# B-R-P/NMSLIB-ZIG

Measured on AMD Instinct MI355X. Metric: queries/sec @ recall@10, 1M x 128-D L2, batch=1024; HBM GB/s vs peak, higher is better.
Workload: dtype f16+f32

## Files before the change

include/nmslib_gpu.h:

```cpp
#ifndef NMSLIB_GPU_H
#define NMSLIB_GPU_H

#include "nmslib_c.h"

#ifdef __cplusplus
extern "C" {
#endif

int nmslib_gpu_device_count(void);

nmslib_error_t nmslib_gpu_finalize(nmslib_index_handle_t index);

nmslib_error_t nmslib_gpu_knn_query_batch_device(nmslib_index_handle_t index,
                                                 const void* d_queries, size_t query_count,
                                                 size_t elem_count, size_t k, int32_t* d_ids,
                                                 float* d_dists, int32_t* d_counts,
                                                 void* stream);

nmslib_error_t nmslib_gpu_last_batch_counters(nmslib_index_handle_t index,
                                              const int32_t** d_ndc, const int32_t** d_hops,
                                              const int32_t** d_hops_up);

nmslib_error_t nmslib_gpu_merge_topk(const float* d_dists_in, const int32_t* d_ids_in,
                                     size_t nshards, size_t query_count, size_t k,
                                     float* d_dists_out, int32_t* d_ids_out, void* stream);

nmslib_error_t nmslib_gpu_merge_topk_strided(const float* d_dists_in, const int32_t* d_ids_in,
                                             size_t shard_stride, size_t nshards, size_t query_count,
                                             size_t k, float* d_dists_out, int32_t* d_ids_out,
                                             void* stream);

nmslib_error_t nmslib_gpu_kernel_timing(nmslib_index_handle_t index, int enable, double* total_ms,
                                        uint64_t* launches);

typedef struct {
    double upload_seconds;
    double build_seconds;
    size_t hbm_bytes;
    size_t rows;
    size_t dim;
    size_t shards;
    size_t last_path;
    size_t fast_tiles;
    size_t fast_tiles_precise;
    size_t fast_tiles_fallback;
    size_t hnsw_redone;
} nmslib_gpu_stats_t;
nmslib_error_t nmslib_gpu_get_stats(nmslib_index_handle_t index, nmslib_gpu_stats_t* out);

nmslib_error_t nmslib_gpu_graph_builder(nmslib_index_handle_t index, int* builder);

nmslib_error_t nmslib_gpu_string_hnsw_links(nmslib_index_handle_t index, size_t node, int level, int32_t* out,
                                            size_t capacity, size_t* count, int* enterpoint, int* maxlevel);

#ifdef __cplusplus
}
#endif
#endif
```

nmslib_zig_amd/__init__.py:

```python
import ctypes as C
import os
import subprocess

import numpy as np

_HERE = os.path.dirname(os.path.abspath(__file__))
LIB_PATH = os.path.join(_HERE, "libnmslib_c.so")

ERRORS = {
    1: "NullPointer", 2: "InvalidArgument", 3: "OutOfMemory", 4: "BufferTooSmall",
    5: "SpaceIncompatible", 6: "QueryTooLarge", 7: "InvalidSparseElement", 8: "IndexBuildFailed",
    9: "QueryExecutionFailed", 10: "DataIOFailed", 11: "PluginRegistrationFailed", 12: "Internal",
    13: "Runtime", 14: "IndexNotBuilt",
}
DATATYPE = {"DenseVector": 0, "SparseVector": 1, "DenseUInt8Vector": 2, "ObjectAsString": 3}
DISTTYPE = {"Float": 0, "Int": 1}
SPARSE_ELEM = np.dtype([("id", "<u4"), ("value", "<f4")])


def sparse_rows(rows):
    if hasattr(rows, "indptr"):
        rows = (rows.indptr, rows.indices, rows.data)
    if isinstance(rows, tuple) and len(rows) == 3 and all(isinstance(a, np.ndarray) for a in rows):
        indptr = np.asarray(rows[0], np.int64)
        el = np.empty(int(indptr[-1] - indptr[0]), SPARSE_ELEM)
        el["id"] = np.asarray(rows[1])[indptr[0]:indptr[-1]]
        el["value"] = np.asarray(rows[2])[indptr[0]:indptr[-1]]
        return el, np.diff(indptr).astype(np.uint64)
    counts = np.array([len(r[0]) for r in rows], np.uint64)
    el = np.empty(int(counts.sum()), SPARSE_ELEM)
    at = 0
    for ids, vals in rows:
        m = len(ids)
        el["id"][at:at + m] = ids
        el["value"][at:at + m] = vals
        at += m
    return el, counts


def _as_bytes(s):
    return s.encode() if isinstance(s, str) else bytes(s)


def sparse_vector(ids, values):
    el = np.empty(len(ids), SPARSE_ELEM)
    el["id"] = ids
    el["value"] = values
    return el


class NmslibError(RuntimeError):
    def __init__(self, code, detail=""):
        self.code = code
        self.name = ERRORS.get(code, "Runtime")
        super().__init__(f"{self.name} ({code}): {detail}")


class Allocator(C.Structure):
    _fields_ = [("alloc", C.CFUNCTYPE(C.c_void_p, C.c_size_t, C.c_void_p)),
                ("free", C.CFUNCTYPE(None, C.c_void_p, C.c_void_p)),
                ("ctx", C.c_void_p)]


class Result(C.Structure):
    _fields_ = [("ids", C.POINTER(C.c_int32)), ("distances", C.POINTER(C.c_float)),
                ("size", C.c_size_t), ("capacity", C.c_size_t)]


class ErrorDetail(C.Structure):
    _fields_ = [("code", C.c_int), ("message", C.c_void_p), ("file", C.c_void_p), ("line", C.c_int)]


class GpuStats(C.Structure):
    _fields_ = [("upload_seconds", C.c_double), ("build_seconds", C.c_double),
                ("hbm_bytes", C.c_size_t), ("rows", C.c_size_t), ("dim", C.c_size_t), ("shards", C.c_size_t),
                ("last_path", C.c_size_t), ("fast_tiles", C.c_size_t), ("fast_tiles_precise", C.c_size_t),
                ("fast_tiles_fallback", C.c_size_t), ("hnsw_redone", C.c_size_t)]


def build_library(force=False):
    csrc = os.path.join(_HERE, "csrc")
    if force:
        subprocess.check_call(["make", "-C", csrc, "clean"], stdout=subprocess.DEVNULL)
    subprocess.check_call(["make", "-C", csrc, "-j8"], stdout=subprocess.DEVNULL)
    return LIB_PATH


_lib = None
_alloc_live = {}


def lib():
    global _lib
    if _lib is not None:
        return _lib
    if not os.path.exists(LIB_PATH):
        raise ImportError(f"{LIB_PATH} is missing: run `python -c 'import __graft_entry__ as g; g.build()'` "
                          "or `make -C nmslib_zig_amd/csrc` (the engine has no CPU fallback)")
    try:
        C.CDLL("libamdhip64.so", mode=C.RTLD_GLOBAL)
    except OSError:
        pass
    L = C.CDLL(LIB_PATH)
    vp, sz, i32p, f32p = C.c_void_p, C.c_size_t, C.POINTER(C.c_int32), C.POINTER(C.c_float)
    AP = C.POINTER(Allocator)
    sigs = {
        "nmslib_init": (None, []),
        "nmslib_index_create": (C.c_int, [C.c_char_p, vp, C.c_char_p, C.c_int, C.c_int, AP, C.POINTER(vp)]),
        "nmslib_index_destroy": (None, [vp]),
        "nmslib_create_index": (C.c_int, [vp, vp, C.c_int]),
        "nmslib_reset_index": (C.c_int, [vp]),
        "nmslib_create_params": (vp, [AP]),
        "nmslib_add_param": (C.c_int, [vp, C.c_char_p, C.c_int, vp]),
        "nmslib_free_params": (None, [vp]),
        "nmslib_get_space_type": (C.c_int, [vp, C.POINTER(vp), C.POINTER(sz), AP]),
        "nmslib_get_method": (C.c_int, [vp, C.POINTER(vp), C.POINTER(sz), AP]),
        "nmslib_free_string": (None, [vp, AP]),
        "nmslib_get_last_error_detail": (C.c_int, [C.POINTER(ErrorDetail), AP]),
        "nmslib_add_data_point": (C.c_int, [vp, vp, sz, C.c_int32]),
        "nmslib_add_data_point_batch": (C.c_int, [vp, vp, sz, sz, vp, vp]),
        "nmslib_add_data_point_batch_uint8": (C.c_int, [vp, vp, sz, sz, vp]),
        "nmslib_add_data_point_batch_string": (C.c_int, [vp, vp, sz, vp]),
        "nmslib_gpu_string_hnsw_links": (C.c_int, [vp, sz, C.c_int, vp, sz, C.POINTER(sz), C.POINTER(C.c_int),
                                                  C.POINTER(C.c_int)]),
        "nmslib_add_data_point_batch_pointers": (C.c_int, [vp, C.c_int, vp, sz, sz, vp, vp]),
        "nmslib_knn_query_get_size": (C.c_int, [vp, vp, sz, sz, C.POINTER(sz), sz]),
        "nmslib_knn_query_fill": (C.c_int, [vp, vp, sz, sz, C.POINTER(Result), sz]),
        "nmslib_knn_query_batch": (C.c_int, [vp, vp, sz, sz, sz, C.POINTER(Result), vp, sz]),
        "nmslib_range_query_get_size": (C.c_int, [vp, vp, sz, C.c_double, C.POINTER(sz), sz]),
        "nmslib_range_query_fill": (C.c_int, [vp, vp, sz, C.c_double, C.POINTER(Result), sz]),
        "nmslib_get_distance": (C.c_int, [vp, sz, sz, C.POINTER(C.c_float)]),
        "nmslib_get_data_point_size": (C.c_int, [vp, sz, C.POINTER(sz)]),
        "nmslib_get_data_point_fill": (C.c_int, [vp, sz, vp, sz]),
        "nmslib_get_data_point_string": (C.c_int, [vp, sz, C.POINTER(vp), C.POINTER(sz), AP]),
        "nmslib_borrow_data_dense": (C.c_int, [vp, sz, C.POINTER(vp), C.POINTER(sz), C.POINTER(vp)]),
        "nmslib_borrow_data_sparse": (C.c_int, [vp, sz, C.POINTER(vp), C.POINTER(sz), C.POINTER(vp)]),
        "nmslib_save_index": (C.c_int, [vp, C.c_char_p, C.c_int]),
        "nmslib_load_index": (C.c_int, [C.c_char_p, C.c_int, C.c_int, AP, C.c_int, C.POINTER(vp)]),
        "nmslib_set_query_time_params": (C.c_int, [vp, vp]),
        "nmslib_set_thread_pool_size": (C.c_int, [vp, sz]),
        "nmslib_get_thread_pool_size": (sz, [vp]),
        "nmslib_data_qty": (sz, [vp]),
        "nmslib_index_memory_usage": (sz, [vp]),
        "nmslib_initialize_pool": (None, [vp]),
        "nmslib_free_result": (None, [C.POINTER(Result), AP]),
        "nmslib_gpu_device_count": (C.c_int, []),
        "nmslib_gpu_finalize": (C.c_int, [vp]),
        "nmslib_gpu_knn_query_batch_device": (C.c_int, [vp, vp, sz, sz, sz, vp, vp, vp, vp]),
        "nmslib_gpu_last_batch_counters": (C.c_int, [vp, C.POINTER(vp), C.POINTER(vp), C.POINTER(vp)]),
        "nmslib_gpu_merge_topk": (C.c_int, [vp, vp, sz, sz, sz, vp, vp, vp]),
        "nmslib_gpu_merge_topk_strided": (C.c_int, [vp, vp, sz, sz, sz, sz, vp, vp, vp]),
        "nmslib_gpu_get_stats": (C.c_int, [vp, C.POINTER(GpuStats)]),
        "nmslib_gpu_kernel_timing": (C.c_int, [vp, C.c_int, C.POINTER(C.c_double), C.POINTER(C.c_uint64)]),
        "nmslib_gpu_graph_builder": (C.c_int, [vp, C.POINTER(C.c_int)]),
    }
    for name, (res, args) in sigs.items():
        fn = getattr(L, name)
        fn.restype = res
        fn.argtypes = args
    _lib = L
# ... 379 lines not shown
```

nmslib_zig_amd/csrc/abi.cpp:

```cpp
#include <cstdio>
#include <cstring>
#include <memory>
#include <new>
#include <thread>
#include <string>
#include <vector>

#include "../../include/nmslib_c.h"
#include "../../include/nmslib_gpu.h"
#include "engine.hpp"

using gfxknn::Engine;
using gfxknn::EngineError;
using gfxknn::Err;

namespace {

struct LastError {
    nmslib_error_t code = NMSLIB_SUCCESS;
    std::string message = "No error";
    std::string file = __FILE__;
    int line = 0;
};
thread_local LastError g_last;
// ... 718 lines not shown
    return n;
}

nmslib_error_t nmslib_gpu_finalize(nmslib_index_handle_t handle) {
    if (!handle) FAIL(NMSLIB_ERROR_INVALID_ARGUMENT, "Invalid index");
    return guarded(NMSLIB_ERROR_INDEX_BUILD_FAILED, "finalize", [&] {
        Engine* e = H(handle)->engine;
        std::lock_guard<std::mutex> lk(e->mu);
        e->finalize();
    });
}

nmslib_error_t nmslib_gpu_knn_query_batch_device(nmslib_index_handle_t handle, const void* d_queries,
                                                 size_t query_count, size_t elem_count, size_t k,
                                                 int32_t* d_ids, float* d_dists, int32_t* d_counts, void* stream) {
    if (!handle || !d_queries || !d_ids || !d_dists || k == 0 || elem_count == 0)
        FAIL(NMSLIB_ERROR_INVALID_ARGUMENT, "Invalid device batch inputs");
    Engine* e = H(handle)->engine;
    if (!e->index_created()) FAIL(NMSLIB_ERROR_INDEX_BUILD_FAILED, "Index not built");
    return guarded(NMSLIB_ERROR_QUERY_EXECUTION_FAILED, "KNN device batch failed", [&] {
        std::lock_guard<std::mutex> lk(e->mu);
        e->knn_device(d_queries, query_count, elem_count, k, d_ids, d_dists, d_counts,
                      static_cast<hipStream_t>(stream));
    });
}

nmslib_error_t nmslib_gpu_last_batch_counters(nmslib_index_handle_t handle, const int32_t** d_ndc,
                                              const int32_t** d_hops, const int32_t** d_hops_up) {
    if (!handle) FAIL(NMSLIB_ERROR_INVALID_ARGUMENT, "Invalid index");
    Engine* e = H(handle)->engine;
    if (d_ndc) *d_ndc = e->last_ndc();
    if (d_hops) *d_hops = e->last_hops();
    if (d_hops_up) *d_hops_up = e->last_hops_up();
    return NMSLIB_SUCCESS;
}

nmslib_error_t nmslib_gpu_merge_topk_strided(const float* d_dists_in, const int32_t* d_ids_in, size_t shard_stride,
                                             size_t nshards, size_t query_count, size_t k, float* d_dists_out,
                                             int32_t* d_ids_out, void* stream) {
    if (!d_dists_in || !d_ids_in || !d_dists_out || !d_ids_out || nshards == 0 || k == 0 || shard_stride < query_count * k)
        FAIL(NMSLIB_ERROR_INVALID_ARGUMENT, "Invalid merge inputs");
    if (nshards * k > 8192) FAIL(NMSLIB_ERROR_QUERY_TOO_LARGE, "nshards * k must not exceed 8192");
    return guarded(NMSLIB_ERROR_RUNTIME, "merge_topk", [&] {
        if (query_count)
            gfxknn::hip_check(gfxknn::launch_merge_topk(d_dists_in, d_ids_in, shard_stride, (int)nshards, (int)query_count,
                                                        (int)k, d_dists_out, d_ids_out, static_cast<hipStream_t>(stream)),
                              "merge_topk");
    });
}

nmslib_error_t nmslib_gpu_merge_topk(const float* d_dists_in, const int32_t* d_ids_in, size_t nshards,
                                     size_t query_count, size_t k, float* d_dists_out, int32_t* d_ids_out,
                                     void* stream) {
    return nmslib_gpu_merge_topk_strided(d_dists_in, d_ids_in, query_count * k, nshards, query_count, k, d_dists_out,
                                         d_ids_out, stream);
}

nmslib_error_t nmslib_gpu_kernel_timing(nmslib_index_handle_t handle, int enable, double* total_ms,
                                        uint64_t* launches) {
    if (!handle) FAIL(NMSLIB_ERROR_INVALID_ARGUMENT, "Invalid index");
    return guarded(NMSLIB_ERROR_RUNTIME, "kernel_timing", [&] {
        Engine* e = H(handle)->engine;
        std::lock_guard<std::mutex> lk(e->mu);
        if (total_ms || launches) e->collect_profile(total_ms, launches);
        e->set_profiling(enable != 0);
    });
}

nmslib_error_t nmslib_gpu_get_stats(nmslib_index_handle_t handle, nmslib_gpu_stats_t* out) {
    if (!handle || !out) FAIL(NMSLIB_ERROR_INVALID_ARGUMENT, "Invalid arguments");
    Engine* e = H(handle)->engine;
    std::memset(out, 0, sizeof(*out));
    return guarded(NMSLIB_ERROR_RUNTIME, "Failed to read statistics", [&] {
        std::lock_guard<std::mutex> lk(e->mu);
        out->upload_seconds = e->upload_seconds;
        out->build_seconds = e->build_seconds;
        out->hbm_bytes = e->hbm_bytes();
        out->rows = e->size();
        out->dim = e->dim();
        out->shards = e->shard_count() ? e->shard_count() : 1;
        out->last_path = (size_t)e->last_path;
        e->fast_tile_counts(&out->fast_tiles, &out->fast_tiles_precise, &out->fast_tiles_fallback);
        out->hnsw_redone = e->hnsw_redone();
    });
}

nmslib_error_t nmslib_gpu_graph_builder(nmslib_index_handle_t handle, int* builder) {
    if (!handle || !builder) FAIL(NMSLIB_ERROR_INVALID_ARGUMENT, "Invalid arguments");
    Engine* e = H(handle)->engine;
    return guarded(NMSLIB_ERROR_RUNTIME, "Failed to read the graph builder", [&] {
        std::lock_guard<std::mutex> lk(e->mu);
        *builder = e->graph_builder();
    });
}

nmslib_error_t nmslib_gpu_string_hnsw_links(nmslib_index_handle_t index, size_t node, int level, int32_t* out,
                                            size_t capacity, size_t* count, int* enterpoint, int* maxlevel) {
    if (!index || !count || !enterpoint || !maxlevel || node >= nmslib_data_qty(index) || level < 0)
        FAIL(NMSLIB_ERROR_INVALID_ARGUMENT, "Invalid graph inputs");
    Engine* e = H(index)->engine;
    if (!e->is_string() || e->method_name() != "hnsw") FAIL(NMSLIB_ERROR_SPACE_INCOMPATIBLE, "Not a string HNSW index");
    if (!e->index_created()) FAIL(NMSLIB_ERROR_INDEX_BUILD_FAILED, "Index not built");
    return guarded(NMSLIB_ERROR_RUNTIME, "Graph inspection", [&] {
        std::lock_guard<std::mutex> lk(e->mu);
        const gfxknn::HostGraph& g = e->string_graph();
        if (level > g.levels[node]) throw EngineError(Err::InvalidArgument, "level above the node's level");
        const int32_t* L = level == 0 ? &g.links0[node * (size_t)(g.maxM0 + 1)]
                                      : &g.up_links[(size_t)g.up_off[node] + (size_t)(level - 1) * (g.maxM + 1)];
        *count = (size_t)L[0];
        *enterpoint = g.enterpoint;
        *maxlevel = g.maxlevel;
        if (out && *count <= capacity) std::memcpy(out, L + 1, *count * sizeof(int32_t));
    });
}

}
```

nmslib_zig_amd/csrc/brute.cpp:

```cpp
#include <algorithm>
#include <cmath>
#include <cstdlib>
#include <cstring>

#include "engine.hpp"
#include "l1_quant.hpp"

namespace gfxknn {

void BruteDense::release() {
    have_bf16 = false;
    have_l1 = false;
    l1_u8.release();
    l1_cols.release();
    bf_hi.release();
    bf_lo.release();
    f16_hi.release();
    auxp.release();
    auxp16.release();
}

size_t BruteDense::bytes() const {
    size_t total = 0;
    for (const DevBuf* b : {&rows_i8, &auxh, &rows_sel, &mean, &bf_hi, &bf_lo, &auxp, &f16_hi, &auxp16, &l1_u8, &l1_cols}) total += b->bytes();
// ... 126 lines not shown
            const double m = st[c] / (double)n;
            mean[c] = (float)m;
            mu2 += m * m;
        }
        const double spread2 = std::max(0.0, st[(size_t)ldb_] / (double)n - mu2);
        b.cosc_spread2 = spread2;
        bool centre = mu2 > 0.0625 * spread2;
        if (const char* env = getenv("NMSLIB_GPU_CENTER")) centre = atoi(env) != 0;
        if (centre) {
            b.mean.ensure((size_t)ldb_ * 4);
            b.rows_sel.ensure(n * (size_t)ldb_ * 4);
            hip_check(hipMemcpyAsync(b.mean.ptr(), mean.data(), (size_t)ldb_ * 4, hipMemcpyHostToDevice, stream_), "mean");
            hip_check(launch_center_rows(d_rows_.as<float>(), b.mean.as<float>(), (int)n, (int)n, ldb_, (int)dim_,
                                         b.rows_sel.as<float>(), stream_),
                      "centre rows");
            hip_check(hipStreamSynchronize(stream_), "centre rows");
            sel_rows = b.rows_sel.as<float>();
            b.centred = true;
            b.mu_norm = 0;
            for (size_t c = 0; c < dim_; ++c) b.mu_norm += (double)mean[c] * (double)mean[c];
            b.mu_norm = std::sqrt(b.mu_norm);
        }
    }
    if (b.centred && space_ != SP_L2) {
        d_aux_.ensure(std::max<size_t>(n, 1) * 12);
        hip_check(launch_row_aux_cosc(d_rows_.as<float>(), sel_rows, (int)n, ldb_, (int)dim_, b.mu_norm, d_aux_.as<float>(),
                                      stream_),
                  "row aux");
    } else {
        hip_check(launch_row_aux_f32(sel_rows, (int)n, ldb_, (int)dim_, space_, d_aux_.as<float>(), stream_), "row aux");
    }
    {
        float bm[4] = {0.f, 0.f, 0.f, 0.f};
        measure_rows_f16(sel_rows, n, ldb_, (int)dim_, cosine, bm);
        b.bmax = bm[0];
        b.bres = bm[1];
    }
    b.release();
    const bool fast_space = space_ == SP_L2 || space_ == SP_NEGDOT || (cosine && !b.centred);
    const int n_pad = bf_f32_rows_padded((int)n);
    if (cosine && b.centred && dim_ + 3 <= 1024 && n >= 65536) {
        const BfF32Fast f0 = bf_f32_fast_plan((int)n, (int)dim_, 1024, 10, space_, true);
        if (f0.use) {
            const size_t dp = (size_t)f0.dp;
            DevBuf d_aug, d_flag;
            d_aug.ensure(n * dp * 4);
            d_flag.ensure(16);
            hip_check(hipMemsetAsync(d_flag.ptr(), 0, 16, stream_), "clear");
            b.cosc_lambda = (float)std::sqrt(std::max(0.5 * b.cosc_spread2, 1e-30));
            hip_check(launch_row_aug_cosc(d_rows_.as<float>(), sel_rows, (int)n, ldb_, (int)dim_, b.mu_norm, b.cosc_lambda,
                                          d_aug.as<float>(), (int)dp, d_flag.as<int>(), stream_),
                      "augmented rows");
            int fl[1] = {0};
            hip_check(hipMemcpyAsync(fl, d_flag.ptr(), 4, hipMemcpyDeviceToHost, stream_), "flags");
            hip_check(hipStreamSynchronize(stream_), "augmented rows");
            if (fl[0] == 0) {
                float bm[4] = {0.f, 0.f, 0.f, 0.f};
                measure_rows_f16(d_aug.as<float>(), n, (int)dp, (int)dim_ + 3, false, bm);
                if (b.mu_norm > 0) {
                    const int eq = std::max(-40, std::min(40, (int)std::lround(std::log2((double)b.f16_scale) - std::log2(b.mu_norm))));
                    b.f16_scale_q = std::ldexp(1.f, eq);
                }
                b.bmax_c = bm[0];
                b.bres_c = bm[1];
                make_fast_tiles({d_aug.as<float>(), (int)n, n_pad, (int)dp, (int)dim_ + 3}, (int)dp, nullptr, 0.f, 1.f);
                hip_check(hipStreamSynchronize(stream_), "split rows");
            }
        }
    }
    if (fast_space && dim_ <= 1024 && n >= 65536) {
        const BfF32Fast f0 = bf_f32_fast_plan((int)n, (int)dim_, 1024, 10, space_, b.centred);
        make_fast_tiles({sel_rows, (int)n, n_pad, ldb_, (int)dim_}, f0.use ? f0.dp : 128,
                        space_ == SP_NEGDOT ? nullptr : d_aux_.as<float>(), space_ == SP_L2 ? -INFINITY : 0.f,
                        space_ == SP_L2 ? b.f16_scale * b.f16_scale : 1.f);
    }
    if (space_ == SP_L1 && n >= 65536 && dim_ <= (size_t)BF_L1_MAX_DIM) make_l1_copy();
    hip_check(hipStreamSynchronize(stream_), "finalize");
}

void Engine::knn_brute(const void* d_queries, size_t nq, size_t k, int32_t* d_ids, float* d_dists, int32_t* d_cnt,
                       hipStream_t stream) {
    BruteDense& b = brute_;
    have_counters_ = false;
    const int dim_eff = d_n_ ? (int)dim_ : 1;
    const BfOut out{d_ids_.as<int32_t>(), d_ids, d_dists, d_cnt};
    if (k > (size_t)BF_MAX_K) {
        const int ld = is_u8() ? 128 : ldb_;
        const int elem = is_u8() ? 1 : 4;
        const size_t n = d_n_;
        ws_qpad_.ensure(std::max<size_t>(nq, 1) * ld * elem);
        hip_check(launch_pad_rows(d_queries, (int)nq, dim_eff, ws_qpad_.ptr(), (int)nq, ld, elem, stream), "pad queries");
        BfBigkWs ws{};
        ws.dist = static_cast<float*>(ws_rdist_.ensure(std::max<size_t>(n, 1) * 4));
        ws.keys = static_cast<uint32_t*>(ws_bigk_.ensure(std::max<size_t>(n, 1) * 16));
        ws.temp_bytes = bf_bigk_temp_bytes((int)n);
        ws.temp = ws_bigk_tmp_.ensure(ws.temp_bytes);
        hip_check(launch_bf_bigk(space_, d_rows_.ptr(), ld, (int)n, dim_eff, ws_qpad_.ptr(), (size_t)ld * elem, (int)nq, (int)k,
                                 ws, out, stream),
                  "bf_bigk");
        last_path = 5;
        return;
    }
    auto fast_ws = [&](const BfFastWsBytes& need) {
        BfFastWs ws{};
        ws.top8 = b.ws_top8.ensure(need.top8);
        ws.thr = b.ws_thr.ensure(need.thr);
        ws.list = static_cast<uint32_t*>(b.ws_list.ensure(need.list));
        ws.list_cnt = static_cast<int*>(b.ws_listcnt.ensure(need.list_cnt));
        ws.fb.cand = static_cast<unsigned long long*>(ws_cand_.ensure(need.cand));
        ws.fb.cnt = static_cast<int*>(ws_cnt_.ensure(need.cnt));
        if (need.flags_fb) ws.flags_fb = static_cast<int*>(b.ws_flags.ensure(need.flags_fb));
        if (need.queries) ws.queries = b.ws_f32_q.ensure(need.queries);
        return ws;
    };
    if (is_u8()) {
        const BfU8Fast f = bf_u8_fast_plan((int)d_n_, (int)nq, (int)k);
        if (f.use) {
            ws_qpad_.ensure((size_t)f.qpad * 128);
            const BfFastWs ws = fast_ws(bf_fast_ws_bytes(f));
            const BfU8Rows rows{d_rows_.as<uint8_t>(), b.rows_i8.as<uint8_t>(), d_aux_.as<int32_t>(), b.auxh.as<int32_t>(), (int)d_n_};
            hip_check(launch_bf_u8_fast(f, (int)nq, (int)k, rows, static_cast<const uint8_t*>(d_queries), ws_qpad_.as<uint8_t>(),
                                        ws, out, prof_pair(), stream),
                      "bf_u8_fast");
            last_path = 3;
            fast_flags_ = ws.tile_fail(f);
            fast_nqt_ = f.nqt;
            fast_has_precise_ = false;
            return;
        }
    }
    const BfF32Rows rows{d_rows_.as<float>(), b.centred ? b.rows_sel.as<float>() : d_rows_.as<float>(), d_aux_.as<float>(),
                         (int)d_n_, dim_eff, d_n_ ? ldb_ : f32_row_stride(dim_eff), b.bmax};
    BfF32Queries q{};
    if (!is_u8() && b.have_bf16) {
        const BfF32Fast f = bf_f32_fast_plan((int)d_n_, dim_eff, (int)nq, (int)k, space_, b.centred);
        if (f.use) {
            const int ldb = ldb_;
            q.padded = static_cast<float*>(ws_qpad_.ensure((size_t)f.qpad * ldb * 4));
            q.sel = q.padded;
            q.scale_q = b.f16_scale_q;
            if (b.centred) {
                hip_check(launch_pad_rows(d_queries, (int)nq, dim_eff, q.padded, f.qpad, ldb, 4, stream), "pad queries");
                ws_qsel_.ensure((size_t)f.qpad * ldb * 4);
                hip_check(launch_center_rows(q.padded, b.mean.as<float>(), f.qpad, (int)nq, ldb, dim_eff, ws_qsel_.as<float>(),
                                             stream),
                          "centre queries");
                q.sel = ws_qsel_.as<float>();
            } else {
                q.raw = static_cast<const float*>(d_queries);
            }
            if (f.cosc) {
                ws_qaux_.ensure((size_t)f.qpad * 16);
                b.ws_qaug.ensure((size_t)f.qpad * f.dp * 4);
                q.centred = ws_qsel_.as<float>();
                q.qaux_cosc = ws_qaux_.as<float>();
                hip_check(launch_query_aux_cosc(q.padded, q.centred, f.qpad, ldb, dim_eff, b.mu_norm, ws_qaux_.as<float>(), stream),
                          "query aux");
                hip_check(launch_query_aug_cosc(q.centred, q.qaux_cosc, (int)nq, f.qpad, ldb, dim_eff, b.cosc_lambda,
                                                b.ws_qaug.as<float>(), f.dp, stream),
                          "augmented queries");
                q.sel = b.ws_qaug.as<float>();
                q.sel_ld = f.dp;
            }
            const BfFastWs ws = fast_ws(bf_fast_ws_bytes(f));
            hip_check(launch_bf_f32_fast(f, space_, (int)nq, (int)k, rows, b.tiles(f.dp, f.cosc), q, ws, out, prof_pair(), stream),
                      "bf_f32_fast");
            last_path = 1;
            fast_flags_ = ws.tile_fail(f);
            fast_nqt_ = f.nqt;
            fast_has_precise_ = true;
            return;
        }
    }
    if (space_ == SP_L1 && b.have_l1) {
        const char* env = getenv("NMSLIB_GPU_L1_FAST");
        const BfL1Fast f = bf_l1_fast_plan((int)d_n_, dim_eff, (int)nq, (int)k);
        if (f.use && !(env && atoi(env) == 0)) {
            ws_qpad_.ensure((size_t)f.qpad * ldb_ * 4);
            BfL1Ws ws{};
            ws.qt = static_cast<uint32_t*>(b.ws_l1_qt.ensure((size_t)f.d4 * f.qpad * 4));
            ws.xe = static_cast<double*>(b.ws_l1_xe.ensure((size_t)f.qpad * 16));
            ws.cand.cand = static_cast<unsigned long long*>(b.ws_l1_cand.ensure((size_t)f.qpad * f.nsplit * f.kprime * 8));
            ws.cand.cnt = static_cast<int*>(b.ws_l1_cnt.ensure((size_t)f.qpad * f.nsplit * 4));
            ws.flags = static_cast<int*>(b.ws_flags.ensure((size_t)f.nqt * 4 + 64));
            ws.fb.cand = static_cast<unsigned long long*>(ws_cand_.ensure(bf_cand_elems(f.fallback) * 8));
            ws.fb.cnt = static_cast<int*>(ws_cnt_.ensure(bf_cnt_elems(f.fallback) * 4));
            const float* cols = b.l1_cols.as<float>();
            const BfL1Rows copy{b.l1_u8.as<uint32_t>(), cols, cols + dim_, cols + 2 * dim_, b.l1_step};
            hip_check(launch_bf_l1_fast(f, (int)nq, (int)k, rows, copy, static_cast<const float*>(d_queries), ws_qpad_.as<float>(),
                                        ws, out, prof_pair(), stream),
                      "bf_l1_fast");
            last_path = 6;
            fast_flags_ = ws.flags;
            fast_nqt_ = f.nqt;
            fast_has_precise_ = false;
            return;
        }
    }
    last_path = is_u8() ? 2 : 0;
    BfPlan p = bf_make_plan((int)d_n_, dim_eff, (int)nq, (int)k, is_u8());
    if (d_n_ == 0) p.ldb = is_u8() ? 128 : f32_row_stride(dim_eff);
    const int elem = is_u8() ? 1 : 4;
    ws_qpad_.ensure((size_t)p.qpad * p.ldb * elem);
    const BfCand c{static_cast<unsigned long long*>(ws_cand_.ensure(bf_cand_elems(p) * 8)),
                   static_cast<int*>(ws_cnt_.ensure(bf_cnt_elems(p) * 4))};
    hip_check(launch_pad_rows(d_queries, (int)nq, dim_eff, ws_qpad_.ptr(), p.qpad, p.ldb, elem, stream), "pad queries");
    q.padded = ws_qpad_.as<float>();
    q.sel = q.padded;
    if (b.centred) {
        ws_qsel_.ensure((size_t)p.qpad * p.ldb * 4);
        hip_check(launch_center_rows(q.padded, b.mean.as<float>(), p.qpad, (int)nq, p.ldb, dim_eff, ws_qsel_.as<float>(), stream),
                  "centre queries");
        q.sel = ws_qsel_.as<float>();
        if (space_ != SP_L2) {
            ws_qaux_.ensure((size_t)p.qpad * 16);
            hip_check(launch_query_aux_cosc(q.padded, q.sel, p.qpad, p.ldb, dim_eff, b.mu_norm, ws_qaux_.as<float>(), stream),
                      "query aux");
            q.qaux_cosc = ws_qaux_.as<float>();
        }
    }
    prof_begin(stream);
    if (is_u8()) {
        hip_check(launch_bf_select_u8(p, b.rows_i8.as<uint8_t>(), d_aux_.as<int32_t>(), ws_qpad_.as<uint8_t>(), c, BfGate{}, stream),
                  "bf_select_u8");
    } else if (space_ == SP_L1 || space_ == SP_LINF) {
        hip_check(launch_bf_select_direct_f32(p, space_, rows.orig, q.padded, c, BfGate{}, stream), "bf_select_direct");
    } else {
        b.ws_flags.ensure((size_t)p.nqt * 4 + 64);
        hip_check(launch_bf_adaptive_f32(p, space_, (int)k, rows, q, c, b.ws_flags.as<int>(), BfGate{}, out, stream),
                  "bf_adaptive_f32");
        prof_end(stream);
        return;
    }
    prof_end(stream);
    hip_check(launch_bf_rerank(p, space_, dim_eff, (int)k, d_rows_.ptr(), ws_qpad_.ptr(), c, BfGate{}, BfVerify{}, out, stream),
              "bf_rerank");
}

}
```

nmslib_zig_amd/csrc/engine.cpp:

```cpp
#include "engine.hpp"
#include "f16_pack.hpp"

#include <algorithm>
#include <chrono>
#include <cmath>
#include <cstring>
#include <fstream>
#include <set>
#include <sstream>
#include <thread>

namespace gfxknn {

using clk = std::chrono::steady_clock;

void hip_check(hipError_t e, const char* what) {
    if (e == hipSuccess) return;
    std::string msg = std::string(what) + ": " + hipGetErrorString(e);
    (void)hipGetLastError();
    throw EngineError(e == hipErrorOutOfMemory ? Err::OutOfMemory : Err::Runtime, msg);
}

ParamSet::ParamSet(const std::vector<std::string>& desc) {
    std::set<std::string> seen;
// ... 210 lines not shown
    if (hipEvent_t a = prof_pair().first) hip_check(hipEventRecord(a, s), "hipEventRecord");
}
void Engine::prof_end(hipStream_t s) {
    if (!prof_ || prof_events_.empty()) return;
    hip_check(hipEventRecord(prof_events_.back().second, s), "hipEventRecord");
}
void Engine::collect_profile(double* total_ms, uint64_t* launches) {
    double tot = 0;
    uint64_t n = 0;
    for (auto& pr : prof_events_) {
        float ms = 0;
        if (hipEventSynchronize(pr.second) == hipSuccess && hipEventElapsedTime(&ms, pr.first, pr.second) == hipSuccess) {
            tot += ms;
            ++n;
        }
        (void)hipEventDestroy(pr.first);
        (void)hipEventDestroy(pr.second);
    }
    prof_events_.clear();
    if (total_ms) *total_ms = tot;
    if (launches) *launches = n;
}

void Engine::add_row(const void* data, size_t elem_count, int32_t id) {
    if (sparse_ || str_space_) throw EngineError(Err::SpaceIncompatible, "Not dense space");
    if (is_u8()) {
        if (elem_count != 128) throw EngineError(Err::Runtime, "SIFT vectors must have 128 bytes");
        if (dim_ == 0) dim_ = 128;
        const uint8_t* p = static_cast<const uint8_t*>(data);
        rows_u8_.insert(rows_u8_.end(), p, p + 128);
    } else {
        if (dim_ == 0) dim_ = elem_count;
        if (elem_count != dim_)
            throw EngineError(Err::InvalidArgument, "all rows of a dense index must have the same dimension");
        const float* p = static_cast<const float*>(data);
        rows_f32_.insert(rows_f32_.end(), p, p + elem_count);
    }
    ids_.push_back(id);
    dirty_ = true;
    graph_dirty_ = true;
}

const void* Engine::host_row(size_t pos) const {
    return is_u8() ? static_cast<const void*>(&rows_u8_[pos * 128]) : static_cast<const void*>(&rows_f32_[pos * dim_]);
}

void Engine::stored_row(size_t pos, void* dst) const {
    if (is_u8()) {
        std::memcpy(dst, &rows_u8_[pos * 128], 128);
        int32_t s = 0;
        for (int i = 0; i < 128; ++i) s += (int32_t)rows_u8_[pos * 128 + i] * (int32_t)rows_u8_[pos * 128 + i];
        std::memcpy(static_cast<char*>(dst) + 128, &s, 4);
    } else {
        std::memcpy(dst, &rows_f32_[pos * dim_], dim_ * 4);
        if (diverg_stores_logs()) diverg_logs(&rows_f32_[pos * dim_], dim_, static_cast<float*>(dst) + dim_);
    }
}

void Engine::reset() {
    ids_.clear();
    rows_f32_.clear();
    rows_u8_.clear();
    sp_ptr_.assign(1, 0);
    sp_ids_.clear();
    sp_vals_.clear();
    st_ptr_.assign(1, 0);
    st_bytes_.clear();
    st_words_.clear();
    st_bits_ = -1;
    graph_ = HostGraph();
    graph_rows_.clear();
    loaded_graph_ = false;
    graph_builder_ = 0;
    created_ = false;
    dirty_ = true;
    graph_dirty_ = true;
    d_n_ = 0;
    shards_.clear();
    dim_ = 0;
    brute_ = BruteDense();
    last_path = 0;
    fast_flags_ = nullptr;
    fast_nqt_ = 0;
    hnsw_fix_valid_ = false;
    have_counters_ = false;
    d_rows16_.release();
    rows16_failed_ = false;
    rows_f16_index_ = rows_f16_ = false;
    rerank_ = 0;
}

size_t Engine::memory_usage() const {
    if (!created_) return 0;
    if (sparse_)
        return ids_.size() * 16 + sp_ids_.size() * sizeof(SparseElem) + hbm_bytes();
    if (str_space_)
        return ids_.size() * 16 + (space_ == SP_LEVEN ? st_bytes_.size() : ids_.size() * (ham_words() + 1) * 4) +
               hbm_bytes();
    size_t total = ids_.size() * (16 + stored_row_bytes());
    total += ids_.size() * dim_ * sizeof(float);
    return total + rows16_bytes();
}

size_t Engine::rows16_bytes() const {
    size_t b = d_rows16_.bytes();
    for (const auto& c : shards_) b += c->rows16_bytes();
    return b;
}

size_t Engine::hbm_bytes() const {
    size_t sh = 0;
    for (const auto& c : shards_) sh += c->hbm_bytes();
    return sh + d_rows_.bytes() + d_aux_.bytes() + d_ids_.bytes() + d_links0_.bytes() + d_up_off_.bytes() + d_up_links_.bytes() +
           d_rownorm_.bytes() + d_rows16_.bytes() + brute_.bytes() + d_sp_ptr_.bytes() + d_sp_ids_.bytes() + d_sp_vals_.bytes() + d_st_ptr_.bytes() + d_st_data_.bytes();
}

void Engine::create_index(const std::vector<std::string>& params) {
    ParamSet ps(params);
    int defer = 0;
    if (method_name_ == "hnsw") {
        method_ = Method::Hnsw;
        HnswBuildParams bp;
        ps.get("M", bp.M);
        int search_method = 0;
        ps.get("searchMethod", search_method);
        ps.get("indexThreadQty", bp.threads);
        ps.get("efConstruction", bp.efConstruction);
        bp.maxM = bp.M;
        ps.get("maxM", bp.maxM);
        bp.maxM0 = bp.M * 2;
        ps.get("maxM0", bp.maxM0);
        ps.get("mult", bp.mult);
        ps.get("delaunay_type", bp.delaunay);
        ps.get("post", bp.post);
        int skip = 0;
        ps.get("skip_optimized_index", skip);
        bp.skip_optimized = skip != 0;
        ps.get("gpu_defer", defer);
        ps.get("gpu_build", bp.gpu_build);
        ps.get("gpu_build_batch", bp.gpu_build_batch);
        ps.get("gpu_build_div", bp.gpu_build_div);
        ps.get("gpu_shards", gpu_shards_);
        std::string gpu_rows = "f32";
        ps.get("gpu_rows", gpu_rows);
        ps.check_unused();
        const bool f16 = parse_gpu_rows(gpu_rows);
        if (f16) check_rows16_served();
        rows_f16_index_ = rows_f16_ = f16;
        rerank_ = 0;
        if (defer && bp.gpu_build < 0) bp.gpu_build = 0;
        bp_ = bp;
        ef_ = 200;
        algo_ = "hybrid";
    } else if (method_name_ == "brute_force" || method_name_ == "seq_search") {
        method_ = Method::Brute;
        bool copy_mem = false, multi = false;
        size_t thread_qty = 0;
        ps.get("copyMem", copy_mem);
        ps.get("multiThread", multi);
        ps.get("threadQty", thread_qty);
        ps.get("gpu_defer", defer);
        ps.get("gpu_shards", gpu_shards_);
        ps.check_unused();
        if ((sparse_ || str_space_ || diverg_) && gpu_shards_ != -1 && gpu_shards_ != 1)
            throw EngineError(Err::IndexBuildFailed, std::string(sparse_ ? "a sparse" : str_space_ ? "a string" : "a divergence") +
                                                         " index runs on one GPU: gpu_shards=" +
// ... 633 lines not shown
            q = c.ws_q_.ptr();
        }
        c.ws_ids_.ensure(nq * k * 4);
        c.ws_dists_.ensure(nq * k * 4);
        c.knn_device(q, nq, elem_count, k, c.ws_ids_.as<int32_t>(), c.ws_dists_.as<float>(), nullptr, c.stream_);
        hip_check(hipMemcpyPeerAsync(ws_sh_ids_.as<int32_t>() + s * nq * k, device_, c.ws_ids_.ptr(), c.device_, nq * k * 4,
                                     c.stream_),
                  "ids P2P");
        hip_check(hipMemcpyPeerAsync(ws_sh_d_.as<float>() + s * nq * k, device_, c.ws_dists_.ptr(), c.device_, nq * k * 4,
                                     c.stream_),
                  "dists P2P");
        hip_check(hipEventRecord(shard_events_[s], c.stream_), "hipEventRecord");
        static const bool serial = getenv("NMSLIB_GPU_SHARD_SERIAL") && atoi(getenv("NMSLIB_GPU_SHARD_SERIAL"));
        if (serial) hip_check(hipStreamSynchronize(c.stream_), "shard (serial)");
    }
    hip_check(hipSetDevice(device_), "hipSetDevice");
    last_path = shards_[0]->last_path;
    for (size_t s = 0; s < S; ++s) hip_check(hipStreamWaitEvent(stream, shard_events_[s], 0), "hipStreamWaitEvent");
    hip_check(launch_merge_topk_ex(ws_sh_d_.as<float>(), ws_sh_ids_.as<int32_t>(), nq * k, (int)S, (int)nq, (int)k, d_dists,
                                   d_ids, d_cnt, d_ids_.as<int32_t>(), stream),
              "merge_topk");
}

void Engine::knn_device(const void* d_queries, size_t nq, size_t elem_count, size_t k, int32_t* d_ids,
                        float* d_dists, int32_t* d_cnt, hipStream_t stream) {
    if (!created_) throw EngineError(Err::IndexBuildFailed, "Index not built");
    if (diverg_)
        throw EngineError(Err::SpaceIncompatible, "the device-resident batch is not served over a divergence space: a "
                                                  "query's logarithms are taken on the host, so divergence queries "
                                                  "go through nmslib_knn_query_batch");
    if (dirty_) finalize();
    check_device();
    if (nq == 0) return;
    if (k == 0) throw EngineError(Err::InvalidArgument, "k must be positive");
    if (sparse_ || str_space_)
        throw EngineError(Err::SpaceIncompatible, "the device-resident batch takes dense queries; sparse and string "
                                                  "queries go through nmslib_knn_query_batch");
    last_stream_ = stream;
    if (!shards_.empty()) {
        if (size() > 0 && elem_count != dim_)
            throw EngineError(Err::QueryExecutionFailed, "query dimension does not match the index");
        knn_sharded(d_queries, nq, elem_count, k, d_ids, d_dists, d_cnt, stream);
        return;
    }
    if (d_n_ > 0 && elem_count != dim_)
        throw EngineError(Err::QueryExecutionFailed, "query dimension does not match the index");
    const size_t slice = method_ == Method::Brute ? 32768 : 65536;
    const size_t qbytes = elem_count * elem_bytes();
    if (method_ == Method::Hnsw) {
        ws_ndc_.ensure(nq * 4);
        ws_hops_.ensure(nq * 4);
        ws_hops_up_.ensure(nq * 4);
        ws_status_.ensure(nq * 4);
    }
    for (size_t q0 = 0; q0 < nq; q0 += slice) {
        const size_t m = std::min(slice, nq - q0);
        ctr_off_ = q0;
        const void* qs = static_cast<const char*>(d_queries) + q0 * qbytes;
        int32_t* cnt = d_cnt ? d_cnt + q0 : nullptr;
        if (method_ == Method::Brute) knn_brute(qs, m, k, d_ids + q0 * k, d_dists + q0 * k, cnt, stream);
        else knn_hnsw(qs, m, k, d_ids + q0 * k, d_dists + q0 * k, cnt, stream);
    }
}

void Engine::fast_tile_counts(size_t* tiles, size_t* precise, size_t* fallback) {
    *tiles = *precise = *fallback = 0;
    if (!shards_.empty()) {
        shards_[0]->fast_tile_counts(tiles, precise, fallback);
        return;
    }
    if ((last_path != 1 && last_path != 3 && last_path != 6) || !fast_flags_ || fast_nqt_ <= 0) return;
    std::vector<int> h((size_t)fast_nqt_ * 2, 0);
    hip_check(hipSetDevice(device_), "hipSetDevice");
    hip_check(hipStreamSynchronize(last_stream_ ? last_stream_ : stream_), "stats");
    hip_check(hipMemcpy(h.data(), fast_flags_, (size_t)fast_nqt_ * (fast_has_precise_ ? 2 : 1) * sizeof(int), hipMemcpyDeviceToHost),
              "stats flags");
    *tiles = (size_t)fast_nqt_;
    for (int i = 0; i < fast_nqt_; ++i) {
        *fallback += h[i] != 0;
        if (fast_has_precise_) *precise += h[(size_t)fast_nqt_ + i] != 0;
    }
}

size_t Engine::hnsw_redone() {
    if (!shards_.empty()) return shards_[0]->hnsw_redone();
    if ((last_path != 4 && last_path != 5) || !hnsw_fix_valid_) return 0;
    int32_t v = 0;
    hip_check(hipSetDevice(device_), "hipSetDevice");
    hip_check(hipStreamSynchronize(last_stream_ ? last_stream_ : stream_), "stats");
    hip_check(hipMemcpy(&v, ws_fix_.ptr(), 4, hipMemcpyDeviceToHost), "stats redo count");
    return (size_t)v;
}

HnswOut Engine::hnsw_out(int32_t* d_ids, float* d_dists, int32_t* d_cnt, size_t nq) {
    if (!d_cnt) {
        ws_outcnt_.ensure(nq * 4);
        d_cnt = ws_outcnt_.as<int32_t>();
    }
    return {d_ids, d_dists, d_cnt, ws_ndc_.as<int32_t>() + ctr_off_, ws_hops_.as<int32_t>() + ctr_off_,
            ws_hops_up_.as<int32_t>() + ctr_off_, ws_status_.as<int32_t>() + ctr_off_};
}

uint32_t* Engine::cleared_bitset(size_t m, size_t words, hipStream_t stream) {
    ws_bitset_.ensure(m * words * 4);
    hip_check(hipMemsetAsync(ws_bitset_.ptr(), 0, m * words * 4, stream), "clear visited bitset");
    return ws_bitset_.as<uint32_t>();
}

void Engine::knn_hnsw(const void* d_queries, size_t nq, size_t k, int32_t* d_ids, float* d_dists, int32_t* d_cnt,
                      hipStream_t stream) {
    const int ef = ef_;
    last_path = 4;
    hnsw_fix_valid_ = false;
    if (search_old()) {
        knn_hnsw_old(d_queries, nq, k, d_ids, d_dists, d_cnt, stream);
        return;
    }
    const HnswOut out = hnsw_out(d_ids, d_dists, d_cnt, nq);
    if (std::max<size_t>(ef, k) > 1024 || hnsw_nbcap(dg_) > HNSW_NBCAP_LDS) {
        const size_t cap = std::max<size_t>(ef, k), words = (d_n_ + 31) / 32;
        const size_t per_q = cap * 8 + words * 4;
        const size_t slice = std::max<size_t>(1, std::min<size_t>(nq, ((size_t)4 << 30) / per_q));
        const size_t qbytes = dim_ * elem_bytes();
        have_counters_ = true;
        for (size_t q0 = 0; q0 < nq; q0 += slice) {
            const size_t m = std::min(slice, nq - q0);
            ws_old_a_.ensure(m * cap * 4);
            ws_old_r_.ensure(m * cap * 4);
            uint32_t* bitset = cleared_bitset(m, words, stream);
            if (q0 == 0) prof_begin(stream);
            hip_check(launch_hnsw_search_big(dg_, (int)m, (int)k, ef, static_cast<const char*>(d_queries) + q0 * qbytes,
                                             bitset, ws_old_a_.as<float>(), ws_old_r_.as<int32_t>(), out.at(q0, k), stream),
                      "hnsw_search(big)");
            if (q0 + slice >= nq) prof_end(stream);
        }
        return;
    }
    if (rows_f16_ && ensure_rows16()) {
        knn_hnsw_f16(d_queries, nq, k, d_ids, d_dists, d_cnt, stream);
        return;
    }
    hnsw_search_lds(dg_, false, d_queries, nq, k, ef, out, true, stream);
}

void Engine::hnsw_search_lds(const HnswDeviceGraph& g, bool rows_f16, const void* d_queries, size_t nq, size_t k, int ef,
                             const HnswOut& out, bool timed, hipStream_t stream) {
    const HnswQueries queries = HnswQueries::external(d_queries);
    HnswSearchPlan p = hnsw_make_plan(g, (int)nq, (int)k, ef, false);
    p.rows_f16 = rows_f16 ? 1 : 0;
    have_counters_ = true;
    if (p.table_size == 0) {
        uint32_t* bitset = cleared_bitset(nq, p.bitset_words, stream);
        prof_begin(stream);
        hip_check(launch_hnsw_search(g, p, queries, bitset, HnswOverflow{}, out, stream), "hnsw_search");
        if (timed) prof_end(stream);
        return;
    }
    const int fix_slots = (int)std::min<size_t>(nq, 128);
    HnswSearchPlan pb = hnsw_make_plan(g, (int)nq, (int)k, ef, true);
    pb.rows_f16 = p.rows_f16;
    ws_fix_.ensure((nq + 16) * 4);
    ws_bitset_.ensure((size_t)fix_slots * pb.bitset_words * 4);
    int32_t* fix_count = ws_fix_.as<int32_t>();
    int32_t* fix_list = fix_count + 16;
    hip_check(hipMemsetAsync(fix_count, 0, 4, stream), "clear overflow count");
    hnsw_fix_valid_ = true;
// ... 535 lines not shown
```

nmslib_zig_amd/csrc/engine.hpp:

```cpp
#pragma once
#include <hip/hip_runtime_api.h>

#include <cstdint>
#include <functional>
#include <map>
#include <memory>
#include <mutex>
#include <stdexcept>
#include <string>
#include <utility>
#include <vector>

#include "kernels/kernels.hpp"

namespace gfxknn {

enum class Err : int {
    InvalidArgument = 2,
    OutOfMemory = 3,
    SpaceIncompatible = 5,
    QueryTooLarge = 6,
    IndexBuildFailed = 8,
    QueryExecutionFailed = 9,
    DataIO = 10,
// ... 111 lines not shown

struct SparseElem {
    uint32_t id;
    float value;
};

class Engine {
   public:
    Engine(const std::string& space, const std::string& method, int data_type, int dist_type,
           const std::vector<std::string>& space_params = {});
    ~Engine();

    const std::string& space_name() const { return space_name_; }
    const std::string& method_name() const { return method_name_; }
    bool is_u8() const { return space_ == SP_L2SQR_SIFT; }
    size_t size() const { return parent_ ? view_n_ : ids_.size(); }
    size_t dim() const { return dim_; }
    size_t elem_bytes() const { return is_u8() ? 1 : 4; }
    size_t row_bytes() const { return dim_ * elem_bytes(); }
    size_t stored_row_bytes() const { return is_u8() ? dim_ + 4 : diverg_stores_logs() ? dim_ * 8 : dim_ * 4; }

    void add_row(const void* data, size_t elem_count, int32_t id);
    const void* host_row(size_t pos) const;
    void stored_row(size_t pos, void* dst) const;
    int32_t ext_id(size_t pos) const { return ids_[pos]; }
    void reset();

    bool is_sparse() const { return sparse_; }
    void add_sparse_row(const SparseElem* elems, size_t count, int32_t id);
    size_t sparse_row_len(size_t pos) const { return (size_t)(sp_ptr_[pos + 1] - sp_ptr_[pos]); }
    void sparse_row(size_t pos, SparseElem* dst) const;
    void knn_sparse_host(const SparseElem* const* queries, const size_t* counts, size_t nq, size_t k,
                         const int32_t** ids, const float** dists, const int32_t** cnt);
    size_t range_sparse_host(const SparseElem* query, size_t count, double radius, size_t capacity, int32_t* ids,
                             float* dists);

    bool diverg_stores_logs() const;
    void diverg_logs(const float* x, size_t count, float* out) const;

    bool is_string() const { return str_space_; }
    const HostGraph& string_graph() {
        ensure_graph();
        return graph_;
    }
    void add_strings(const char* const* strs, const size_t* lens, size_t count, const int32_t* ids);
    size_t string_object_bytes(size_t pos) const;
    std::string string_object(size_t pos) const;
    void knn_string_host(const char* const* queries, const size_t* lens, size_t nq, size_t k, const int32_t** ids,
                         const float** dists, const int32_t** cnt);
    size_t range_string_host(const char* query, size_t len, double radius, size_t capacity, int32_t* ids, float* dists);

    void create_index(const std::vector<std::string>& params);
    void set_query_params(const std::vector<std::string>& params);
    bool index_created() const { return created_; }
    void finalize();

    void knn_device(const void* d_queries, size_t nq, size_t elem_count, size_t k, int32_t* d_ids,
                    float* d_dists, int32_t* d_cnt, hipStream_t stream);
    void knn_host(const void* queries, size_t nq, size_t elem_count, size_t k, const int32_t** ids, const float** dists,
                  const int32_t** cnt);
    float pair_distance(size_t p1, size_t p2);
    size_t range_host(const void* query, size_t elem_count, double radius, size_t capacity, int32_t* ids, float* dists);
    bool is_brute() const { return method_ == Method::Brute; }

    void save(const std::string& path, bool save_data);
    static std::unique_ptr<Engine> load(const std::string& path, int data_type, int dist_type, bool load_data);

    size_t thread_pool_size = 0;
    size_t memory_usage() const;

    const int32_t* last_ndc() const { return have_counters_ ? ws_ndc_.as<int32_t>() : nullptr; }
    const int32_t* last_hops() const { return have_counters_ ? ws_hops_.as<int32_t>() : nullptr; }
    const int32_t* last_hops_up() const { return have_counters_ ? ws_hops_up_.as<int32_t>() : nullptr; }

    void set_profiling(bool on) { prof_ = on; }
    void collect_profile(double* total_ms, uint64_t* launches);

    double upload_seconds = 0, build_seconds = 0;
    int last_path = 0;
    size_t rows16_bytes() const;
    const int* fast_flags_ = nullptr;
    int fast_nqt_ = 0;
    bool fast_has_precise_ = false;
    void fast_tile_counts(size_t* tiles, size_t* precise, size_t* fallback);
    size_t hnsw_redone();
    hipStream_t last_stream_ = nullptr;
    bool hnsw_fix_valid_ = false;
    size_t hbm_bytes() const;

    std::mutex mu;

    size_t shard_count() const { return shards_.size(); }
    int graph_builder() const { return shards_.empty() ? graph_builder_ : shards_[0]->graph_builder_; }

   private:
    const float* rows_f32() const { return parent_ ? parent_->rows_f32_.data() + view_lo_ * dim_ : rows_f32_.data(); }
    const uint8_t* rows_u8() const { return parent_ ? parent_->rows_u8_.data() + view_lo_ * 128 : rows_u8_.data(); }
    int resolve_shards() const;
    void finalize_sharded(int nshards);
    void knn_sharded(const void* d_queries, size_t nq, size_t elem_count, size_t k, int32_t* d_ids, float* d_dists,
                     int32_t* d_cnt, hipStream_t stream);
    std::vector<std::unique_ptr<Engine>> shards_;
    std::vector<hipEvent_t> shard_events_;
    hipEvent_t shard_ready_ = nullptr;
    const Engine* parent_ = nullptr;
    size_t view_lo_ = 0, view_n_ = 0;
    int forced_device_ = -1;
    int gpu_shards_ = -1;
    DevBuf ws_sh_ids_, ws_sh_d_, ws_bigk_, ws_bigk_tmp_;
    void* pinned(size_t bytes);
    void* pinned_ = nullptr;
    size_t pinned_bytes_ = 0;
    void check_device();
    struct ResultBlock {
        int32_t* ids;
        float* dists;
        int32_t* cnt;
    };
    ResultBlock result_block(size_t nq, size_t k);
    void fetch_results(size_t nq, size_t k, const char* what, const int32_t** ids, const float** dists,
                       const int32_t** cnt);
    using ScanLaunch = std::function<void(const ScanPlan& p, size_t q0, float* split_d, int32_t* split_pos)>;
    void scan_slices(size_t nq, size_t k, int tq, const ResultBlock& out, const ScanLaunch& launch);
    using RangeLaunch = std::function<void(float* filter, float* report)>;
    size_t range_select(bool two_dists, float r, size_t capacity, int32_t* ids, float* dists, const RangeLaunch& launch);
    float read_float(const float* d_out, const char* what);
    void upload_sparse();
    float pair_distance_sparse(size_t p1, size_t p2);
    void upload_diverg();
    DivergRows diverg_rows() const;
    void knn_diverg_host(const float* queries, size_t nq, size_t elem_count, size_t k, const int32_t** ids,
                         const float** dists, const int32_t** cnt);
    size_t range_diverg_host(const float* query, size_t elem_count, double radius, size_t capacity, int32_t* ids,
                             float* dists);
    float pair_distance_diverg(size_t p1, size_t p2);
    void upload_strings();
    void build_string_graph();
    void knn_string_hnsw(const int64_t* d_qoff, const int32_t* d_qlen, const uint64_t* d_peq, const uint32_t* d_qw,
                         int nw_max, size_t nq, size_t k, int32_t* d_ids, float* d_dists, int32_t* d_cnt);
    float pair_distance_string(size_t p1, size_t p2);
    static bool parse_bits(const char* s, size_t len, std::vector<uint32_t>& words, size_t& bits);
    void string_query(const char* s, size_t len, Err parse_err, std::vector<uint32_t>& words) const;
    size_t ham_words() const { return st_bits_ > 0 ? (size_t)(st_bits_ + 31) / 32 : 0; }
    void ensure_graph();
    void upload_rows();
    void build_graph();
    bool use_gpu_build() const;
    void build_graph_gpu();
    void build_graph_gpu_pass(const std::vector<int32_t>& levels, bool reverse);
    void prepare_graph_rows();
    void upload_graph();
    void prepare_brute();
    void measure_rows_f16(const float* rows, size_t n, int ld, int dim, bool relative, float* bm);
    void make_fast_tiles(const BfSplitSrc& src, int dp, const float* aux, float aux_pad, float aux16_mul);
    void make_l1_copy();
    void knn_brute(const void* d_queries, size_t nq, size_t k, int32_t* d_ids, float* d_dists,
                   int32_t* d_cnt, hipStream_t stream);
    void knn_hnsw(const void* d_queries, size_t nq, size_t k, int32_t* d_ids, float* d_dists,
                  int32_t* d_cnt, hipStream_t stream);
    void knn_hnsw_old(const void* d_queries, size_t nq, size_t k, int32_t* d_ids, float* d_dists,
                      int32_t* d_cnt, hipStream_t stream);
    bool search_old() const { return algo_ == "old" || (algo_ == "hybrid" && ef_ >= 1000); }
    void hnsw_search_lds(const HnswDeviceGraph& g, bool rows_f16, const void* d_queries, size_t nq, size_t k, int ef,
                         const HnswOut& out, bool timed, hipStream_t stream);
    void knn_hnsw_f16(const void* d_queries, size_t nq, size_t k, int32_t* d_ids, float* d_dists, int32_t* d_cnt,
                      hipStream_t stream);
// ... 70 lines not shown
```

nmslib_zig_amd/csrc/kernels/bf_kernels.hip:

```cpp
#include <cstdio>
#include <type_traits>
#include <vector>
#include <cstdlib>

#include "common_dev.hpp"
#include "kernels.hpp"

namespace gfxknn {

enum BfMode : int { BF_L2 = 0, BF_DOT = 1, BF_COS = 2, BF_L1 = 3, BF_LINF = 4, BF_COSC = 5, BF_L2D = 6 };

struct BfArgs {
    const float* base;
    const float* aux;
    const float* qaux;
    int aux_stride;
    const float* queries;
    u64* cand;
    int* cand_cnt;
    uint32_t* gthr;
    uint32_t* gq;
    int xj, xm;
    int n, ldb, nqt, nsplit, rows_per_split, kprime, cap;
    int kcs;
    int nchunks;
    int dbg;
    const int* tile_fail;
    int fail_group;
};

__device__ __forceinline__ int acc_row(int r, int h) { return (r & 3) + 8 * (r >> 2) + 4 * h; }

__device__ __forceinline__ u64 wave_max_u64(u64 v) {
#pragma unroll
    for (int o = 32; o > 0; o >>= 1) {
        const u64 other = __shfl_xor(v, o, 64);
        v = other > v ? other : v;
    }
    return v;
}

__device__ __forceinline__ void wave_sort128_u64(u64& k0, u64& k1, int lane) {
#pragma unroll
    for (int k2 = 2; k2 <= 128; k2 <<= 1) {
        const bool asc = ((2 * lane) & k2) == 0;
#pragma unroll
        for (int j = k2 >> 1; j >= 1; j >>= 1) {
            if (j == 1) {
                const u64 lo = k0 < k1 ? k0 : k1, hi = k0 < k1 ? k1 : k0;
                k0 = asc ? lo : hi;
                k1 = asc ? hi : lo;
            } else {
                const int lj = j >> 1;
                const bool keep_min = ((lane & lj) == 0) == asc;
                const u64 o0 = __shfl_xor(k0, lj, 64), o1 = __shfl_xor(k1, lj, 64);
                k0 = keep_min ? (o0 < k0 ? o0 : k0) : (o0 > k0 ? o0 : k0);
                k1 = keep_min ? (o1 < k1 ? o1 : k1) : (o1 > k1 ? o1 : k1);
            }
        }
    }
}

__device__ __forceinline__ u64 gather_key(const u64* g, int idx, int n0, int n1, int half) {
    if (idx < n0) return g[idx];
    if (idx - n0 < n1) return g[half + idx - n0];
    return 0ull;
}

__device__ __forceinline__ uint32_t compact_small(u64* g, int n0, int n1, int half, int kprime, int lane,
                                                  int* keep_out) {
    const int n = n0 + n1;
    u64 r0 = gather_key(g, lane, n0, n1, half);
    u64 r1 = gather_key(g, lane + 64, n0, n1, half);
    u64 r2 = gather_key(g, lane + 128, n0, n1, half);
    u64 r3 = gather_key(g, lane + 192, n0, n1, half);
    const int keep = n < kprime ? n : kprime;
    u64 mine = 0ull;
    for (int t = 0; t < keep; ++t) {
        const u64 a01 = r0 > r1 ? r0 : r1, a23 = r2 > r3 ? r2 : r3;
        const u64 w = wave_max_u64(a01 > a23 ? a01 : a23);
        r0 = r0 == w ? 0ull : r0;
        r1 = r1 == w ? 0ull : r1;
// ... 26 lines not shown
    const u64 m = __ballot(need);
    const int lane = threadIdx.x & 63;
    return ((m | (m >> 32) | (m << 32)) >> lane) & 1ull;
}

__device__ __forceinline__ uint32_t compact_queries(u64* gbase , size_t qstride, int cap,
                                                    int kprime, u64* scratch, bool need, int& mycnt, int lane) {
    const int half = cap >> 1, l31 = lane & 31;
    if (__any(need)) {
        const int n_other = __shfl_xor(mycnt, 32, 64);
        const bool fits = need_pair(need) && (mycnt + n_other <= kprime);
        if (fits) {
            if (lane >= 32) {
                u64* g = gbase + (size_t)l31 * qstride;
                for (int i = 0; i < mycnt; ++i) g[n_other + i] = g[half + i];
                mycnt = 0;
            } else {
                mycnt += n_other;
            }
            need = false;
        }
    }
    u64 m = __ballot(need);
    m = (m | (m >> 32)) & 0xFFFFFFFFull;
    uint32_t my_thr = 0u;
    if (m) {
        __builtin_amdgcn_fence(__ATOMIC_RELEASE, "workgroup");
        __builtin_amdgcn_fence(__ATOMIC_ACQUIRE, "workgroup");
    }
    while (m) {
        const int q = __ffsll((long long)m) - 1;
        m &= m - 1;
        const int n0 = __shfl(mycnt, q, 64), n1 = __shfl(mycnt, q + 32, 64);
        u64* g = gbase + (size_t)q * qstride;
        int keep;
        uint32_t t;
        if (cap <= 256 && kprime <= 32) t = compact_small(g, n0, n1, half, kprime, lane, &keep);
        else t = compact_sort(g, n0, n1, half, kprime, scratch, lane, &keep);
        if (l31 == q) {
            mycnt = (lane < 32) ? keep : 0;
            my_thr = t;
        }
    }
    return my_thr;
}

__device__ __forceinline__ uint32_t counted_bound(uint32_t* row, int nsplit, int split, int h, uint32_t pu,
                                                  int xm) {
    if (h == 0) __hip_atomic_store(row + split, pu, __ATOMIC_RELAXED, __HIP_MEMORY_SCOPE_AGENT);
    uint32_t tm[8];
#pragma unroll
    for (int i = 0; i < 8; ++i) tm[i] = 0u;
    auto ins = [&](uint32_t v) __attribute__((always_inline)) {
#pragma unroll
        for (int i = 0; i < 8; ++i) {
            const uint32_t hi = tm[i] > v ? tm[i] : v;
            v = tm[i] > v ? v : tm[i];
            tm[i] = hi;
        }
    };
    const int per = nsplit >> 2;
    const u64* r64 = reinterpret_cast<const u64*>(row) + h * per;
    for (int i = 0; i < per; ++i) {
        const u64 w = __hip_atomic_load(r64 + i, __ATOMIC_RELAXED, __HIP_MEMORY_SCOPE_AGENT);
        const int s0 = 2 * (h * per + i);
        ins(s0 == split ? pu : (uint32_t)w);
        ins(s0 + 1 == split ? pu : (uint32_t)(w >> 32));
    }
    uint32_t o[8];
#pragma unroll
    for (int i = 0; i < 8; ++i) o[i] = __shfl_xor(tm[i], 32, 64);
#pragma unroll
    for (int i = 0; i < 8; ++i) ins(o[i]);
    uint32_t t = tm[0];
#pragma unroll
    for (int i = 1; i < 8; ++i) t = (i == xm - 1) ? tm[i] : t;
    return t;
}

__device__ long long g_bf_clk[2];
__device__ long long g_bf_trace[2048][3];

template <int MODE, bool FULL, bool ONE>
__global__ __launch_bounds__(256, 2) void bf_select_f32_kernel(BfArgs a) {
    extern __shared__ __attribute__((aligned(16))) char smem[];
    const int tid = threadIdx.x, lane = tid & 63, wave = tid >> 6;
    const long long clk_c0 = __builtin_readcyclecounter(), clk_r0 = wall_clock64();
    const int h = lane >> 5, l31 = lane & 31;

    const int b = blockIdx.x;
    const int xcd = b & 7, rest = b >> 3;
    const int qt = rest % a.nqt;
    const int split = (rest / a.nqt) * 8 + xcd;
    if (split >= a.nsplit) return;
    if (a.tile_fail && a.tile_fail[qt / a.fail_group] == 0) return;

    constexpr bool kDirect = (MODE == BF_L1 || MODE == BF_LINF || MODE == BF_L2D);
    constexpr bool kDelay = !kDirect;
    constexpr bool kCosC = (MODE == BF_COSC);
    constexpr int kAuxN = kCosC ? 3 : 1;
    constexpr bool kAux = (MODE == BF_L2 || MODE == BF_COS || kCosC);

    const int kcs = FULL ? BF_KC : a.kcs;
    const int lds_stride = kcs + 4;
    float* tile = reinterpret_cast<float*>(smem);
    float* auxs = tile + 2 * BF_BN * lds_stride;
    u64* scratch = reinterpret_cast<u64*>(auxs + 4 * BF_BN * 3) + (size_t)wave * a.cap;

    const int qidx = qt * BF_TQ + wave * 32 + l31;
    const int half = a.cap >> 1;
    u64* candq = a.cand + ((size_t)qidx * a.nsplit + split) * a.cap + (size_t)h * half;
    int mycnt = 0;
    u64* wave_cand = a.cand + ((size_t)(qt * BF_TQ + wave * 32) * a.nsplit + split) * a.cap;
    const size_t qstride = (size_t)a.nsplit * a.cap;
    const bool use_top8 = a.kprime <= 16;
    const bool track8 = use_top8 || a.xj > 0;
    float t8[8];
#pragma unroll
    for (int i = 0; i < 8; ++i) t8[i] = -INFINITY;
    float thr = -INFINITY;

    const int r_begin = split * a.rows_per_split;
    const int r_end = min(a.n, r_begin + a.rows_per_split);
    const int nstages = r_end > r_begin ? (r_end - r_begin + BF_BN - 1) / BF_BN : 0;
    const int nchunks = ONE ? 1 : a.nchunks;
    const int nsteps = nstages * nchunks;

    const int sc = tid & 31, sr = tid >> 5;
    f32x4 stg[8];
    float stg_aux[kAuxN];
    float cq2 = 0.f, cqnp = 0.f, cqn = 0.f, cqf = 1.f;

    auto issue_loads = [&](int step) __attribute__((always_inline)) {
        const int stage = step / nchunks, kc = step - stage * nchunks;
        const int row0 = r_begin + stage * BF_BN;
        const int col0 = kc * BF_KC + sc * 4;
        const int kc_len = FULL ? BF_KC : min(kcs, a.ldb - kc * BF_KC);
#pragma unroll
        for (int i = 0; i < 8; ++i) {
            const int row = row0 + sr + 8 * i;
            f32x4 v = {0.f, 0.f, 0.f, 0.f};
            if (sc * 4 < kc_len && row < r_end)
                v = *reinterpret_cast<const f32x4*>(a.base + (size_t)row * a.ldb + col0);
            stg[i] = v;
        }
        if (kAux && kc == 0 && tid < BF_BN) {
            const int row = row0 + tid;
            stg_aux[0] = row < r_end ? a.aux[row] : -INFINITY;
            if constexpr (kCosC) {
                stg_aux[1] = row < r_end ? a.aux[(size_t)a.aux_stride + row] : 0.f;
                stg_aux[2] = row < r_end ? a.aux[2 * (size_t)a.aux_stride + row] : 1.f;
            }
        }
    };
    auto write_lds = [&](int step) __attribute__((always_inline)) {
        const int stage = step / nchunks, kc = step - stage * nchunks;
        float* t = tile + (step & 1) * BF_BN * lds_stride;
        if (sc * 4 < kcs) {
#pragma unroll
            for (int i = 0; i < 8; ++i)
                *reinterpret_cast<f32x4*>(t + (sr + 8 * i) * lds_stride + sc * 4) = stg[i];
        }
        if (kAux && kc == 0 && tid < BF_BN) {
#pragma unroll
            for (int c = 0; c < kAuxN; ++c) auxs[((stage % 3) * kAuxN + c) * BF_BN + tid] = stg_aux[c];
        }
    };

    auto write_lds_piece = [&](int step, int i) __attribute__((always_inline)) {
        float* t = tile + (step & 1) * BF_BN * lds_stride;
        if (sc * 4 < kcs) *reinterpret_cast<f32x4*>(t + (sr + 8 * i) * lds_stride + sc * 4) = stg[i];
    };
    auto write_lds_aux = [&](int step) __attribute__((always_inline)) {
// ... 229 lines not shown
        const f32x4 qa = *reinterpret_cast<const f32x4*>(a.qaux + (size_t)qidx * 4);
        cq2 = qa[0];
        cqnp = qa[1];
        cqn = qa[2];
        cqf = qa[3];
    }
    if (nchunks == 1) {
        load_queries(0);
        __builtin_amdgcn_s_waitcnt(0x0F70);
        spread_queries();
    }
    __syncthreads();

    const bool skip_epi = (a.dbg & 1) != 0;
    const int xmask = (a.dbg >> 12) ? ((1 << ((a.dbg >> 12) & 7)) - 1) : 3;
    for (int step = 0; step < nsteps; ++step) {
        const int stage = step / nchunks, kc = step - stage * nchunks;
        const bool have_next = step + 1 < nsteps;
        if (have_next && !((a.dbg & 2) && step > 0)) issue_loads(step + 1);
        if (!ONE && nchunks > 1) {
            load_queries(kc);
            spread_queries();
        }
        const int kc_len = FULL ? BF_KC : min(kcs, a.ldb - kc * BF_KC);
        const float* t = tile + (step & 1) * BF_BN * lds_stride;
        const bool first = kc == 0, lastc = kc == nchunks - 1;
        if constexpr (!kDirect) {
            const float* ap0 = t + l31 * lds_stride + 4 * h;
            if (first) {
#pragma unroll
                for (int i = 0; i < 16; ++i) accX[i] = 0.f;
            }
            f32x4 fr0 = *reinterpret_cast<const f32x4*>(ap0), fr1 = fr0;
            if (8 < kc_len) fr1 = *reinterpret_cast<const f32x4*>(ap0 + 8);
            block_mfma(accX, ap0, ap0 + 32 * lds_stride, fr0, fr1, kc_len, first && stage > 0 && !skip_epi, accY, 1,
                       stage - 1, -1);
            if (lastc) add_norm(accX, 0, stage);
            if (first) {
#pragma unroll
                for (int i = 0; i < 16; ++i) accY[i] = 0.f;
            }
            const bool stage_next = have_next && !((a.dbg & 2) && step > 0);
            block_mfma(accY, ap0 + 32 * lds_stride, nullptr, fr0, fr1, kc_len, lastc && !skip_epi, accX, 0, stage,
                       (FULL && stage_next) ? step + 1 : -1);
            if (lastc) add_norm(accY, 1, stage);
            if (skip_epi) asm volatile("" ::"v"(accX[0]), "v"(accY[0]), "v"(accX[15]), "v"(accY[15]));
        } else {
            if (first) {
#pragma unroll
                for (int i = 0; i < 16; ++i) {
                    accX[i] = 0.f;
                    accY[i] = 0.f;
                }
            }
            block_direct(accX, t, 0, kc_len);
            block_direct(accY, t, 1, kc_len);
            if (lastc && !skip_epi) {
                check_block(accX, 0, stage);
                check_block(accY, 1, stage);
                if (stage == nstages - 1) {
                    if (a.xj > 0 && !(a.dbg & (256 | 512))) exchange_counted();
                    finish_stage(true);
                }
            }
        }
        if ((!FULL || kDirect) && have_next && !((a.dbg & 2) && step > 0)) write_lds(step + 1);
        flush_pending();
        if (lastc && !(a.dbg & 256)) {
            if (a.xj > 0 && !(a.dbg & 512)) {
                if ((stage & (stage + 1)) == 0 || (stage & 31) == 31) exchange_counted();
            } else if ((stage & xmask) == xmask) {
                exchange_thr();
            }
        }
        if (!(a.dbg & 8)) __syncthreads();
    }
    if (kDelay && nstages > 0 && !skip_epi) {
        check_block(accY, 1, nstages - 1);
        if (a.xj > 0 && !(a.dbg & (256 | 512))) exchange_counted();
        if (!(a.dbg & 16)) finish_stage(true);
    }
    if (h == 0) a.cand_cnt[(size_t)qidx * a.nsplit + split] = mycnt;
    if ((a.dbg & 1024) && tid == 0) {
        if (blockIdx.x == 0) {
            g_bf_clk[0] = __builtin_readcyclecounter() - clk_c0;
            g_bf_clk[1] = wall_clock64() - clk_r0;
        }
        if (blockIdx.x < 2048) {
            g_bf_trace[blockIdx.x][0] = clk_r0;
            g_bf_trace[blockIdx.x][1] = wall_clock64();
            g_bf_trace[blockIdx.x][2] = __builtin_amdgcn_s_getreg((4 << 0) | (0 << 6) | (31 << 11));
        }
    }
}

struct BfArgsU8 {
    const uint8_t* base_i8;
    const int32_t* aux;
    const uint8_t* queries;
    u64* cand;
    int* cand_cnt;
    uint32_t* gq;
    int xj, xm;
    int n, nqt, nsplit, rows_per_split, kprime, cap;
    int dbg;
    int tile_stride;
    const int* tile_fail;
    int fail_group;
};

typedef const __attribute__((address_space(1))) void* gptr_t;
typedef __attribute__((address_space(3))) void* lptr_t;

__global__ __launch_bounds__(256, 2) void bf_select_u8_kernel(BfArgsU8 a) {
    extern __shared__ __attribute__((aligned(16))) char smem[];
    const int tid = threadIdx.x, lane = tid & 63, wave = tid >> 6;
    const int h = lane >> 5, l31 = lane & 31;
    const int b = blockIdx.x;
    const int xcd = b & 7, rest = b >> 3;
    const int qt = rest % a.nqt;
    const int split = (rest / a.nqt) * 8 + xcd;
    if (split >= a.nsplit) return;
    if (a.tile_fail && a.tile_fail[qt / a.fail_group] == 0) return;

    constexpr int kRing = 6, kAuxRing = 8, kTileBytes = BF_BN * 128;
    constexpr int kThr0 = -(1 << 29);
    char* ring = smem;
    int* auxr = reinterpret_cast<int*>(ring + kRing * kTileBytes);
    u64* scratch = reinterpret_cast<u64*>(auxr + kAuxRing * BF_BN) + (size_t)wave * a.cap;

    const int qidx = qt * BF_TQ + wave * 32 + l31;
    const int half = a.cap >> 1;
    u64* candq = a.cand + ((size_t)qidx * a.nsplit + split) * a.cap + (size_t)h * half;
    int mycnt = 0;
    u64* wave_cand = a.cand + ((size_t)(qt * BF_TQ + wave * 32) * a.nsplit + split) * a.cap;
    const size_t qstride = (size_t)a.nsplit * a.cap;

    const int tstr = a.tile_stride;
    const int tps = a.rows_per_split / BF_BN;
    const int tiles_all = (a.n + BF_BN - 1) / BF_BN;
    const int stiles_all = (tiles_all + tstr - 1) / tstr;
    const int nstages = max(0, min(tps, stiles_all - split * tps));
    const int r_begin = split * tps * tstr * BF_BN;
    const int stage_rows = tstr * BF_BN;

    const int dma_row = lane >> 3;
    auto issue_tile = [&](int stage) __attribute__((always_inline)) {
        const int slot = stage % kRing;
        const int row0 = r_begin + stage * stage_rows;
#pragma unroll
        for (int jj = 0; jj < 2; ++jj) {
            const int j = 2 * wave + jj;
            const int row = 8 * j + dma_row;
            const int c = (lane & 7) ^ ((row >> 1) & 7);
            const uint8_t* src = a.base_i8 + (size_t)(row0 + row) * 128 + c * 16;
            __builtin_amdgcn_global_load_lds((gptr_t)src, (lptr_t)(ring + slot * kTileBytes + j * 1024), 16, 0, 0);
        }
        if (lane < 16)
            __builtin_amdgcn_global_load_lds((gptr_t)(a.aux + row0 + 16 * wave + lane),
                                             (lptr_t)(auxr + (stage % kAuxRing) * BF_BN + 16 * wave), 4, 0, 0);
    };

    i32x4 bq[4];
#pragma unroll
    for (int ks = 0; ks < 4; ++ks) {
        i32x4 v = *reinterpret_cast<const i32x4*>(a.queries + (size_t)qidx * 128 + 32 * ks + 16 * h);
        bq[ks] = v ^ (int)0x80808080;
    }
    __builtin_amdgcn_s_waitcnt(0x0F70);

    const bool use_top8 = a.kprime <= 16;
    const bool track8 = use_top8 || a.xj > 0;
    int t8[8];
#pragma unroll
    for (int i = 0; i < 8; ++i) t8[i] = INT32_MIN;
    int thr = kThr0;
// ... 1657 lines not shown
            } else {
                sk = (a.space == SP_ANGULAR ? cosf(dk) : 1.0f - dk) * qn;
                e = 6.1036e-5f * qn;
            }
            const float t = fmaxf(s_thr, s_cut);
            if (!split_product) {
                const float unit = a.scale * a.scale_q;
                sk *= unit;
                extra *= unit;
                e = s_e1;
            }
            e += extra + 1e-6f * (fabsf(sk) + fabsf(t));
            if (!(sk - t >= e)) atomicOr(&a.tile_fail[q / a.fail_queries], 1);
        }
    }
    lap(4);
    for (int i = tid; i < a.k; i += blockDim.x) {
        int32_t id = -1;
        float d = INFINITY;
        if (i < found) {
            const u64 key = keys[i];
            const uint32_t pos = (uint32_t)key;
            id = a.ext_ids ? a.ext_ids[pos] : (int32_t)pos;
            d = ord_f32((uint32_t)(key >> 32));
        }
        a.out_ids[(size_t)q * a.k + i] = id;
        a.out_dists[(size_t)q * a.k + i] = d;
    }
    if (tid == 0 && a.out_cnt) a.out_cnt[q] = found;
    lap(5);
}

__global__ void row_maxnorm_kernel(const float* rows, int n, int ld, int dim, int relative, unsigned* out_bits, float scale16) {
    const int lane = threadIdx.x & 63;
    const int wpb = blockDim.x >> 6;
    float mb = 0.f, mr = 0.f, ma = 0.f, mh = 0.f;
    for (int row = blockIdx.x * wpb + (threadIdx.x >> 6); row < n; row += gridDim.x * wpb) {
        const float* p = rows + (size_t)row * ld;
        float s = 0.f, r = 0.f, rh = 0.f;
        for (int d = lane; d < dim; d += 64) {
            const float v = p[d], w = v - (float)(__bf16)v;
            const float vs = scale16 * v, wh = vs - (float)(_Float16)vs;
            s = fmaf(v, v, s);
            r = fmaf(w, w, r);
            rh = fmaf(wh, wh, rh);
            ma = fmaxf(ma, fabsf(v));
        }
        s = wave_sum(s);
        r = wave_sum(r);
        rh = wave_sum(rh);
        const float nb = sqrtf(s), nr = sqrtf(r), nh = sqrtf(rh);
        mb = fmaxf(mb, nb);
        mr = fmaxf(mr, relative ? (nb > 0.f ? nr / nb : 0.f) : nr);
        mh = fmaxf(mh, relative ? (nb > 0.f ? nh / nb : 0.f) : nh);
    }
    ma = wave_max(ma);
    if (lane == 0) {
        atomicMax(out_bits, __float_as_uint(mb));
        atomicMax(out_bits + 1, __float_as_uint(mr));
        atomicMax(out_bits + 2, __float_as_uint(ma));
        atomicMax(out_bits + 3, __float_as_uint(mh));
    }
}

struct RerankArgs {
    const void* base;
    const void* queries;
    const u64* cand;
    const int* cand_cnt;
    const int32_t* ext_ids;
    int32_t* out_ids;
    float* out_dists;
    int32_t* out_cnt;
    int space, dim, ldb, k, nsplit, cap, kprime, p2max;
    const int* tile_fail;
    int fail_queries;
    int* verify_flags;
    int verify_queries;
    const float* queries_sel;
    float bmax;
    float eps_rel;
};

__global__ __launch_bounds__(256) void bf_rerank_kernel(RerankArgs a) {
    extern __shared__ __attribute__((aligned(16))) char smem[];
    u64* keys = reinterpret_cast<u64*>(smem);
    int* offs = reinterpret_cast<int*>(keys + a.p2max);
    const int q = blockIdx.x, tid = threadIdx.x, lane = tid & 63, wave = tid >> 6;
    if (a.tile_fail && a.tile_fail[q / a.fail_queries] == 0) return;

    if (tid == 0) {
        int o = 0;
        for (int s = 0; s < a.nsplit; ++s) {
            offs[s] = o;
            int c = a.cand_cnt[(size_t)q * a.nsplit + s];
            o += c < a.kprime ? c : a.kprime;
        }
        offs[a.nsplit] = o;
    }
    __syncthreads();
    const int total = offs[a.nsplit];
    __shared__ uint32_t s_kth;
    const bool verify = a.verify_flags != nullptr && a.space == SP_L2 && total >= a.kprime;
    if (tid == 0) s_kth = 0xffffffffu;
    for (int idx = tid; idx < a.nsplit * a.kprime; idx += blockDim.x) {
        const int s = idx / a.kprime, i = idx - s * a.kprime;
        const int c = offs[s + 1] - offs[s];
        if (i < c) keys[offs[s] + i] = a.cand[((size_t)q * a.nsplit + s) * a.cap + i];
    }
    __syncthreads();
    if (verify) {
        for (int i = tid; i < total; i += blockDim.x) {
            const uint32_t si = (uint32_t)(keys[i] >> 32);
            int above = 0;
            for (int j = 0; j < total; ++j) above += (uint32_t)(keys[j] >> 32) > si;
            if (above < a.kprime) atomicMin(&s_kth, si);
        }
    }
    __syncthreads();
    for (int i = tid; i < total; i += blockDim.x) keys[i] = (u64)sel_key_pos(keys[i]);
    __syncthreads();
    const int P = next_pow2(total < 2 ? 2 : total);
    if (a.space != SP_L2SQR_SIFT && a.dim <= 256) {
        const float* qq = reinterpret_cast<const float*>(a.queries) + (size_t)q * a.ldb;
        for (int j0 = wave * 4; j0 < total; j0 += 16) {
            uint32_t pos[4];
            const float* rows[4];
#pragma unroll
            for (int r = 0; r < 4; ++r) {
                const int j = j0 + r < total ? j0 + r : total - 1;
                pos[r] = (uint32_t)keys[j];
                rows[r] = reinterpret_cast<const float*>(a.base) + (size_t)pos[r] * a.ldb;
            }
            float d[4];
            wave_exact_distance_f32_x4(a.space, rows, qq, a.dim, lane, d);
            __builtin_amdgcn_wave_barrier();
#pragma unroll
            for (int r = 0; r < 4; ++r)
                if (lane == 0 && j0 + r < total) keys[j0 + r] = ((u64)f32_ord(d[r]) << 32) | pos[r];
        }
    } else {
        for (int j = wave; j < total; j += 4) {
            const uint32_t pos = (uint32_t)keys[j];
            u64 key;
            if (a.space == SP_L2SQR_SIFT) {
                const uint8_t* row = reinterpret_cast<const uint8_t*>(a.base) + (size_t)pos * 128;
                const uint8_t* qq = reinterpret_cast<const uint8_t*>(a.queries) + (size_t)q * 128;
                const int d = wave_exact_distance_u8(row, qq, lane);
                key = ((u64)i32_ord(d) << 32) | pos;
            } else {
                const float* row = reinterpret_cast<const float*>(a.base) + (size_t)pos * a.ldb;
                const float* qq = reinterpret_cast<const float*>(a.queries) + (size_t)q * a.ldb;
                const float d = wave_exact_distance_f32(a.space, row, qq, a.dim, lane);
                key = ((u64)f32_ord(d) << 32) | pos;
            }
            __builtin_amdgcn_wave_barrier();
            if (lane == 0) keys[j] = key;
        }
    }
    for (int i = total + tid; i < P; i += blockDim.x) keys[i] = ~0ull;
    __syncthreads();
    block_bitonic_u64_asc(keys, P, tid, blockDim.x);
    const int found = total < a.k ? total : a.k;
    for (int i = tid; i < a.k; i += blockDim.x) {
        int32_t id = -1;
        float d = INFINITY;
        if (i < found) {
            const u64 key = keys[i];
            const uint32_t pos = (uint32_t)key;
            id = a.ext_ids ? a.ext_ids[pos] : (int32_t)pos;
            d = (a.space == SP_L2SQR_SIFT) ? (float)ord_i32((uint32_t)(key >> 32))
                                           : ord_f32((uint32_t)(key >> 32));
        }
        a.out_ids[(size_t)q * a.k + i] = id;
        a.out_dists[(size_t)q * a.k + i] = d;
    }
    if (tid == 0 && a.out_cnt) a.out_cnt[q] = found;
    if (verify && found > 0) {
        __shared__ float s_qn2v;
        if (tid < 64) {
            const float* qs = a.queries_sel + (size_t)q * a.ldb;
            float ss = 0.f;
            for (int d = tid; d < a.dim; d += 64) ss = fmaf(qs[d], qs[d], ss);
            ss = wave_sum(ss);
            if (tid == 0) s_qn2v = ss;
        }
        __syncthreads();
        if (tid == 0) {
            const float qn2 = s_qn2v, qn = sqrtf(qn2);
            const float kth = ord_f32(s_kth);
            const float dk = ord_f32((uint32_t)(keys[found - 1] >> 32));
            const float e = a.eps_rel * (qn * a.bmax + 0.5f * a.bmax * a.bmax);
            const float floor_d2 = qn2 - 2.0f * kth - 2.0f * e - 2e-6f * (qn2 + fabsf(kth));
            if (!(dk * dk <= floor_d2)) atomicOr(&a.verify_flags[q / a.verify_queries], 1);
        }
    }
}

__global__ void row_aux_f32_kernel(const float* base, int n, int ldb, int dim, int space, float* aux) {
    const int lane = threadIdx.x & 63;
    const int row = blockIdx.x * (blockDim.x >> 6) + (threadIdx.x >> 6);
    if (row >= n) return;
    const float* p = base + (size_t)row * ldb;
    float s = 0.f;
    for (int d = lane; d < dim; d += 64) s = fmaf(p[d], p[d], s);
    s = wave_sum(s);
    if (lane == 0) {
        float v = 0.f;
        if (space == SP_L2) v = -0.5f * s;
        else if (space == SP_COSINE || space == SP_ANGULAR)
            v = (s < 1.17549435e-38f * 2.0f) ? 0.f : 1.0f / sqrtf(s);
        aux[row] = v;
    }
}

__global__ void prepare_u8_kernel(const uint8_t* base, int n, int n_pad, uint8_t* rows_i8, int32_t* aux, int32_t* auxh) {
    const int lane = threadIdx.x & 63;
    const int row = blockIdx.x * (blockDim.x >> 6) + (threadIdx.x >> 6);
    if (row >= n_pad) return;
    uint16_t* dst = reinterpret_cast<uint16_t*>(rows_i8 + (size_t)row * 128);
    if (row >= n) {
        dst[lane] = 0;
        if (lane == 0) {
            aux[row] = -(1 << 30);
            if (auxh) auxh[row] = -(1 << 29);
        }
        return;
    }
    const uint8_t* p = base + (size_t)row * 128;
    const int x0 = p[2 * lane], x1 = p[2 * lane + 1];
    dst[lane] = (uint16_t)((x0 | (x1 << 8)) ^ 0x8080);
    const int sum = wave_sum_i(x0 + x1);
    const int sq = wave_sum_i(x0 * x0 + x1 * x1);
    if (lane == 0) {
        aux[row] = 256 * sum - sq;
        if (auxh) auxh[row] = (256 * sum - sq) >> 1;
    }
}

__global__ void pad_rows_kernel(const uint8_t* src, int rows, int row_bytes, uint8_t* dst, int rows_pad,
                                int ld_bytes) {
    const size_t total = (size_t)rows_pad * ld_bytes;
    for (size_t i = (size_t)blockIdx.x * blockDim.x + threadIdx.x; i < total;
         i += (size_t)gridDim.x * blockDim.x) {
        const size_t r = i / ld_bytes, c = i - r * ld_bytes;
        dst[i] = (r < (size_t)rows && c < (size_t)row_bytes) ? src[r * row_bytes + c] : (uint8_t)0;
    }
}

__global__ void bf_u8_prep_kernel(const uint8_t* raw, int nq, uint8_t* padded, int qpad, int* clr0, int n0, uint32_t* clr1,
                                  size_t n1) {
    const size_t gtid = (size_t)blockIdx.x * blockDim.x + threadIdx.x, gsz = (size_t)gridDim.x * blockDim.x;
    if ((reinterpret_cast<uintptr_t>(raw) & 3) == 0) {
        const size_t words = (size_t)qpad * 32;
        const uint32_t* src = reinterpret_cast<const uint32_t*>(raw);
        uint32_t* dst = reinterpret_cast<uint32_t*>(padded);
        for (size_t i = gtid; i < words; i += gsz) dst[i] = i < (size_t)nq * 32 ? src[i] : 0u;
    } else {
        const size_t bytes = (size_t)qpad * 128;
        for (size_t i = gtid; i < bytes; i += gsz) padded[i] = i < (size_t)nq * 128 ? raw[i] : (uint8_t)0;
    }
    for (size_t i = gtid; i < (size_t)n0; i += gsz) clr0[i] = 0;
    for (size_t i = gtid; i < n1; i += gsz) clr1[i] = 0u;
}

__global__ void normalize_rows_kernel(float* rows, int n, int ld, int dim) {
    const int lane = threadIdx.x & 63;
    const int row = blockIdx.x * (blockDim.x >> 6) + (threadIdx.x >> 6);
    if (row >= n) return;
    float* p = rows + (size_t)row * ld;
    float s = 0.f;
    for (int d = lane; d < dim; d += 64) s = fmaf(p[d], p[d], s);
    s = wave_sum(s);
    if (s != 0.0f) {
        const float inv = 1.0f / sqrtf(s);
        for (int d = lane; d < dim; d += 64) p[d] *= inv;
    }
// ... 145 lines not shown
        d = wave_exact_distance_f32(space, (const float*)a, (const float*)b, dim, lane);
    if (lane == 0) *out = d;
}

__global__ void merge_topk_kernel(const float* dists_in, const int32_t* ids_in, size_t shard_stride, int nshards,
                                  int nq, int k, float* dists_out, int32_t* ids_out, int32_t* cnt_out,
                                  const int32_t* ext_ids) {
    extern __shared__ __attribute__((aligned(16))) char smem[];
    u64* keys = reinterpret_cast<u64*>(smem);
    const int q = blockIdx.x, tid = threadIdx.x;
    const int total = nshards * k;
    const int P = next_pow2(total < 2 ? 2 : total);
    for (int i = tid; i < P; i += blockDim.x) {
        u64 key = ~0ull;
        if (i < total) {
            const int s = i / k, j = i - s * k;
            const size_t off = (size_t)s * shard_stride + (size_t)q * k + j;
            const int32_t id = ids_in[off];
            if (id >= 0) key = ((u64)f32_ord(dists_in[off]) << 32) | (uint32_t)id;
        }
        keys[i] = key;
    }
    __syncthreads();
    block_bitonic_u64_asc(keys, P, tid, blockDim.x);
    for (int i = tid; i < k; i += blockDim.x) {
        const u64 key = keys[i];
        const bool ok = key != ~0ull;
        const int32_t id = (int32_t)(uint32_t)key;
        ids_out[(size_t)q * k + i] = ok ? (ext_ids ? ext_ids[id] : id) : -1;
        dists_out[(size_t)q * k + i] = ok ? ord_f32((uint32_t)(key >> 32)) : INFINITY;
    }
    if (cnt_out && tid == 0) {
        int c = 0;
        while (c < k && keys[c] != ~0ull) ++c;
        cnt_out[q] = c;
    }
}

__global__ void merge_topk_big_kernel(const float* dists_in, const int32_t* ids_in, size_t shard_stride, int nshards,
                                      int nq, int k, float* dists_out, int32_t* ids_out, int32_t* cnt_out,
                                      const int32_t* ext_ids) {
    const int q = blockIdx.x;
    auto key_of = [&](int s, int j) -> u64 {
        const size_t off = (size_t)s * shard_stride + (size_t)q * k + j;
        const int32_t id = ids_in[off];
        return id >= 0 ? (((u64)f32_ord(dists_in[off]) << 32) | (uint32_t)id) : ~0ull;
    };
    for (int i = threadIdx.x; i < k; i += blockDim.x) {
        ids_out[(size_t)q * k + i] = -1;
        dists_out[(size_t)q * k + i] = INFINITY;
    }
    __syncthreads();
    int valid = 0;
    for (int i = threadIdx.x; i < nshards * k; i += blockDim.x) {
        const int s = i / k, j = i - s * k;
        const u64 key = key_of(s, j);
        if (key == ~0ull) continue;
        valid++;
        int rank = j;
        for (int t = 0; t < nshards && rank < k; ++t) {
            if (t == s) continue;
            int lo = 0, hi = k;
            while (lo < hi) {
                const int mid = (lo + hi) >> 1;
                if (key_of(t, mid) < key) lo = mid + 1;
                else hi = mid;
            }
            rank += lo;
        }
        if (rank < k) {
            const int32_t id = (int32_t)(uint32_t)key;
            ids_out[(size_t)q * k + rank] = ext_ids ? ext_ids[id] : id;
            dists_out[(size_t)q * k + rank] = ord_f32((uint32_t)(key >> 32));
        }
    }
    if (cnt_out) {
        __shared__ int total;
        if (threadIdx.x == 0) total = 0;
        __syncthreads();
        atomicAdd(&total, valid);
        __syncthreads();
        if (threadIdx.x == 0) cnt_out[q] = total < k ? total : k;
    }
}

static int host_next_pow2(int v) {
    int p = 1;
    while (p < v) p <<= 1;
    return p;
}

BfPlan bf_make_plan(int n, int dim, int nq, int k, bool is_u8, int qpad_multiple) {
    BfPlan p{};
    p.nq = nq;
    p.qpad = (nq + qpad_multiple - 1) / qpad_multiple * qpad_multiple;
    p.nqt = p.qpad / BF_TQ;
    p.n = n;
    p.ldb = is_u8 ? 128 : f32_row_stride(dim);
    p.kprime = is_u8 ? k : k + (k / 8 > 4 ? k / 8 : 4);
    p.cap = host_next_pow2(2 * p.kprime + BF_BN);
    if (p.cap < 256) p.cap = 256;
    int want = (512 + p.nqt - 1) / p.nqt;
    int by_rows = (n + 2 * BF_BN - 1) / (2 * BF_BN);
    int by_sort = 4096 / p.kprime;
    int ns = want < by_rows ? want : by_rows;
    if (ns > by_sort) ns = by_sort;
    const int ns_cap = p.nqt <= 2 ? 256 : 64;
    if (ns > ns_cap) ns = ns_cap;
    if (const char* e = getenv("NMSLIB_GPU_SPLITS")) ns = atoi(e);
    ns = (ns + 7) / 8 * 8;
    if (ns < 8) ns = 8;
    p.nsplit = ns;
    int rps = (n + ns - 1) / ns;
    p.rows_per_split = (rps + BF_BN - 1) / BF_BN * BF_BN;
    if (p.rows_per_split < BF_BN) p.rows_per_split = BF_BN;
    p.p2max = host_next_pow2(p.nsplit * p.kprime);
    {
        int m = (p.kprime + 1) / 2;
        if (m > 8) m = 8;
        if (m > p.nsplit * 3 / 4) m = p.nsplit * 3 / 4;
        if (m < 1) m = 1;
        const int jj = (p.kprime + 2 * m - 1) / (2 * m);
        p.xm = m;
        p.xj = jj <= 8 ? jj : 0;
    }
    const int kcs = p.ldb < BF_KC ? p.ldb : BF_KC;
    if (is_u8)
        p.lds_select = 6 * BF_BN * 128 + 8 * BF_BN * 4 + 4 * (size_t)p.cap * 8;
    else
        p.lds_select = (size_t)2 * BF_BN * (kcs + 4) * 4 + 4 * BF_BN * 3 * 4 + 4 * (size_t)p.cap * 8;
    p.lds_rerank = (size_t)p.p2max * 8 + (p.nsplit + 1) * 4 + 16;
    return p;
}

template <int MODE, bool FULL, bool ONE>
static hipError_t launch_select_kern(const BfPlan& p, const BfArgs& a, hipStream_t s) {
    auto kern = bf_select_f32_kernel<MODE, FULL, ONE>;
    hipError_t e = hipFuncSetAttribute(reinterpret_cast<const void*>(kern),
                                       hipFuncAttributeMaxDynamicSharedMemorySize, (int)p.lds_select);
    if (e != hipSuccess) return e;
    const int grid = 8 * p.nqt * (p.nsplit / 8);
    hipLaunchKernelGGL(kern, dim3(grid), dim3(256), p.lds_select, s, a);
    if (a.dbg & 1024) {
        long long h[2] = {0, 0};
        (void)hipStreamSynchronize(s);
        (void)hipMemcpyFromSymbol(h, HIP_SYMBOL(g_bf_clk), sizeof(h));
        fprintf(stderr, "[bf_select] block 0: %lld shader cycles, %.1f us, %.0f MHz\n", h[0], h[1] / 100.0,
                h[1] ? (double)h[0] / (h[1] / 100.0) : 0.0);
        static long long tr[2048][3];
        (void)hipMemcpyFromSymbol(tr, HIP_SYMBOL(g_bf_trace), sizeof(tr));
        const int nb = grid < 2048 ? grid : 2048;
        long long t0 = tr[0][0];
        for (int i = 0; i < nb; ++i) t0 = tr[i][0] < t0 ? tr[i][0] : t0;
        if (getenv("NMSLIB_GPU_TRACE") && grid >= 512) {
            FILE* f = fopen(getenv("NMSLIB_GPU_TRACE"), "w");
            if (f) {
                for (int i = 0; i < nb; ++i)
                    fprintf(f, "%d %.2f %.2f %llx\n", i, (tr[i][0] - t0) / 100.0, (tr[i][1] - t0) / 100.0,
                            (unsigned long long)tr[i][2]);
                fclose(f);
            }
        }
    }
    return hipGetLastError();
}

template <int MODE>
static hipError_t launch_select_mode(const BfPlan& p, const BfArgs& a, hipStream_t s) {
#ifdef BF_FAST_COMPILE
    if (MODE == BF_L2 && p.ldb == BF_KC) return launch_select_kern<BF_L2, true, true>(p, a, s);
    return hipErrorInvalidValue;
#else
    if constexpr (MODE == BF_L1 || MODE == BF_LINF || MODE == BF_L2D) {
        return launch_select_kern<MODE, false, false>(p, a, s);
    } else {
        if (p.ldb == BF_KC) return launch_select_kern<MODE, true, true>(p, a, s);
        if (p.ldb % BF_KC == 0) return launch_select_kern<MODE, true, false>(p, a, s);
        return launch_select_kern<MODE, false, false>(p, a, s);
    }
#endif
}

static BfArgs make_args(const BfPlan& p, const float* base, const float* aux, const float* q, const BfCand& c,
                        const BfGate& gate, uint32_t* gthr) {
    BfArgs a{};
    a.base = base;
    a.aux = aux;
    a.queries = q;
    a.cand = c.cand;
    a.cand_cnt = c.cnt;
    a.tile_fail = gate.flags;
    a.fail_group = gate.tiles;
    a.gthr = gthr;
    a.gq = gthr + p.qpad;
    a.xj = p.xj;
    a.xm = p.xm;
    a.n = p.n;
    a.ldb = p.ldb;
    a.nqt = p.nqt;
    a.nsplit = p.nsplit;
    a.rows_per_split = p.rows_per_split;
    a.kprime = p.kprime;
    a.cap = p.cap;
    a.kcs = p.ldb < BF_KC ? p.ldb : BF_KC;
    a.nchunks = (p.ldb + BF_KC - 1) / BF_KC;
    static const int dbg = getenv("NMSLIB_GPU_DEBUG") ? atoi(getenv("NMSLIB_GPU_DEBUG")) : 0;
    a.dbg = dbg;
    return a;
}

static hipError_t select_f32(const BfPlan& p, int space, const float* base, const float* aux, const float* queries_padded,
                             const float* qaux_cosc, const BfCand& c, const BfGate& gate, hipStream_t s, bool cleared) {
    uint32_t* gthr = reinterpret_cast<uint32_t*>(c.cnt + (size_t)p.qpad * p.nsplit);
    if (!cleared) {
        hipError_t me = hipMemsetAsync(gthr, 0, ((size_t)p.qpad + (size_t)p.qpad * p.nsplit) * 4, s);
        if (me != hipSuccess) return me;
    }
    BfArgs a = make_args(p, base, aux, queries_padded, c, gate, gthr);
    switch (space) {
        case SP_L2: return launch_select_mode<BF_L2>(p, a, s);
        case SP_NEGDOT: return launch_select_mode<BF_DOT>(p, a, s);
        case SP_COSINE:
        case SP_ANGULAR:
            if (qaux_cosc) {
                a.qaux = qaux_cosc;
                a.aux_stride = p.n;
                return launch_select_mode<BF_COSC>(p, a, s);
            }
            return launch_select_mode<BF_COS>(p, a, s);
        default: return hipErrorInvalidValue;
    }
}

hipError_t launch_bf_select_direct_f32(const BfPlan& p, int space, const float* base, const float* queries_padded,
                                       const BfCand& c, const BfGate& gate, hipStream_t s, bool cleared_second_region) {
    const size_t gwords = (size_t)p.qpad + (size_t)p.qpad * p.nsplit;
    uint32_t* gthr = reinterpret_cast<uint32_t*>(c.cnt + (size_t)p.qpad * p.nsplit);
    if (cleared_second_region) {
        gthr += gwords;
    } else {
        hipError_t me = hipMemsetAsync(gthr, 0, gwords * 4, s);
        if (me != hipSuccess) return me;
    }
    BfArgs a = make_args(p, base, nullptr, queries_padded, c, gate, gthr);
    if (space == SP_L1) return launch_select_mode<BF_L1>(p, a, s);
    if (space == SP_LINF) return launch_select_mode<BF_LINF>(p, a, s);
    if (space == SP_L2) return launch_select_mode<BF_L2D>(p, a, s);
    return hipErrorInvalidValue;
}

hipError_t launch_bf_select_u8(const BfPlan& p, const uint8_t* base_i8, const int32_t* aux, const uint8_t* queries_padded,
                               const BfCand& c, const BfGate& gate, hipStream_t s, bool cleared) {
    BfArgsU8 a{};
    a.tile_stride = 1;
    a.tile_fail = gate.flags;
    a.fail_group = gate.tiles;
    a.base_i8 = base_i8;
    a.aux = aux;
    a.queries = queries_padded;
    a.cand = c.cand;
    a.cand_cnt = c.cnt;
    a.n = p.n;
    a.nqt = p.nqt;
    a.nsplit = p.nsplit;
    a.rows_per_split = p.rows_per_split;
    a.kprime = p.kprime;
    a.cap = p.cap;
    uint32_t* gthr = reinterpret_cast<uint32_t*>(c.cnt + (size_t)p.qpad * p.nsplit);
    a.gq = gthr + p.qpad;
    a.xj = p.xj;
    a.xm = p.xm;
    static const int dbg = getenv("NMSLIB_GPU_DEBUG") ? atoi(getenv("NMSLIB_GPU_DEBUG")) : 0;
    a.dbg = dbg;
    if (!cleared) {
        hipError_t me = hipMemsetAsync(gthr, 0, ((size_t)p.qpad + (size_t)p.qpad * p.nsplit) * 4, s);
        if (me != hipSuccess) return me;
    }
    hipError_t e = hipFuncSetAttribute(reinterpret_cast<const void*>(bf_select_u8_kernel),
                                       hipFuncAttributeMaxDynamicSharedMemorySize, (int)p.lds_select);
    if (e != hipSuccess) return e;
    const int grid = 8 * p.nqt * (p.nsplit / 8);
    hipLaunchKernelGGL(bf_select_u8_kernel, dim3(grid), dim3(256), p.lds_select, s, a);
    return hipGetLastError();
}

hipError_t launch_bf_rerank(const BfPlan& p, int space, int dim, int k, const void* base, const void* queries_padded,
                            const BfCand& c, const BfGate& gate, const BfVerify& verify, const BfOut& out, hipStream_t s) {
    RerankArgs a{};
    a.verify_flags = verify.flags;
    a.verify_queries = BF_TQ;
    a.queries_sel = verify.queries_sel;
    a.bmax = verify.bmax;
    a.eps_rel = 1.5f * (float)(dim + 2) * 5.9604645e-8f;
    a.tile_fail = gate.flags;
    a.fail_queries = gate.tiles * BF_TQ;
    a.base = base;
    a.queries = queries_padded;
    a.cand = c.cand;
    a.cand_cnt = c.cnt;
    a.ext_ids = out.ext_ids;
    a.out_ids = out.ids;
    a.out_dists = out.dists;
    a.out_cnt = out.cnt;
    a.space = space;
    a.dim = dim;
    a.ldb = p.ldb;
    a.k = k;
    a.nsplit = p.nsplit;
    a.cap = p.cap;
    a.kprime = p.kprime;
    a.p2max = p.p2max;
    hipError_t e = hipFuncSetAttribute(reinterpret_cast<const void*>(bf_rerank_kernel),
                                       hipFuncAttributeMaxDynamicSharedMemorySize, (int)p.lds_rerank);
    if (e != hipSuccess) return e;
    hipLaunchKernelGGL(bf_rerank_kernel, dim3(p.nq), dim3(256), p.lds_rerank, s, a);
    return hipGetLastError();
}

hipError_t launch_bf_adaptive_f32(const BfPlan& p, int space, int k, const BfF32Rows& rows, const BfF32Queries& q,
                                  const BfCand& c, int* flags, const BfGate& gate, const BfOut& out, hipStream_t s,
                                  bool cleared) {
    hipError_t e = select_f32(p, space, rows.sel, rows.aux, q.sel, q.qaux_cosc, c, gate, s, cleared);
    if (e != hipSuccess) return e;
    const bool verify = space == SP_L2 && flags != nullptr && rows.bmax > 0.f;
    if (!verify) return launch_bf_rerank(p, space, rows.dim, k, rows.orig, q.padded, c, gate, BfVerify{}, out, s);
    if (!cleared) {
        e = hipMemsetAsync(flags, 0, (size_t)p.nqt * 4, s);
        if (e != hipSuccess) return e;
    }
    e = launch_bf_rerank(p, space, rows.dim, k, rows.orig, q.padded, c, gate, BfVerify{flags, q.sel, rows.bmax}, out, s);
    if (e != hipSuccess) return e;
    const BfGate failed{flags, 1};
    e = launch_bf_select_direct_f32(p, SP_L2, rows.orig, q.padded, c, failed, s, cleared);
    if (e != hipSuccess) return e;
    return launch_bf_rerank(p, space, rows.dim, k, rows.orig, q.padded, c, failed, BfVerify{}, out, s);
}

BfU8Fast bf_u8_fast_plan(int n, int nq, int k) {
    BfU8Fast f{};
    f.use = (n >= 65536 && nq >= 512 && k <= 256);
    if (const char* e = getenv("NMSLIB_GPU_U8_FAST")) f.use = f.use && atoi(e) != 0;
    if (!f.use) return f;
    f.qg = nq >= 2048 ? 4 : 2;
    const int tq = BF_TQ * f.qg;
    f.qpad = (nq + tq - 1) / tq * tq;
    f.nqt = f.qpad / tq;
    f.stride = 8;
    if (const char* e = getenv("NMSLIB_GPU_U8_STRIDE")) f.stride = atoi(e) > 0 ? atoi(e) : 8;
    const double kf = (double)k / f.stride;
    f.r = (int)(1.6 * kf + 3.0 * sqrt(kf) + 3.0 + 0.999);
    const int tiles_all = (n + BF_BN - 1) / BF_BN;
    int ns = (512 + f.nqt - 1) / f.nqt;
    if (ns > tiles_all / 16) ns = tiles_all / 16;
    if (ns > 256) ns = 256;
    ns = (ns + 7) / 8 * 8;
    if (ns < 8) ns = 8;
    while ((tiles_all + ns - 1) / ns > 32768) ns += 8;
    f.nsplit = ns;
    f.tps = (tiles_all + ns - 1) / ns;
    const double mean_half = (double)f.r * f.stride / (2.0 * ns);
    int caph = 8;
    while (caph < 4.0 * mean_half + 8.0) caph <<= 1;
    f.caph = caph;
    f.p2max = host_next_pow2(2 * ns * caph);
    f.lds_scan = 8 * BF_BN * 128 + 8 * BF_BN * 4 + 64;
    f.lds_rerank = (size_t)f.p2max * 8 + (2 * (size_t)ns + 1) * 4 + 16;
    const int stiles = (tiles_all + f.stride - 1) / f.stride;
    const int s_nqt = f.qpad / (BF_TQ * f.qg);
    int nss = (256 + s_nqt - 1) / s_nqt;
    if (nss > stiles / 32) nss = stiles / 32;
    if (nss > 64) nss = 64;
    nss = (nss + 7) / 8 * 8;
    if (nss < 8) nss = 8;
    f.s_nsplit = nss;
    f.s_tps = (stiles + nss - 1) / nss;
    f.lds_thr = (size_t)host_next_pow2(nss * 2 * 8) * 8 + 16;
    f.fallback = bf_make_plan(n, 128, nq, k, true, tq);
    return f;
}

hipError_t launch_bf_u8_fast(const BfU8Fast& f, int nq, int k, const BfU8Rows& rows, const uint8_t* queries_raw,
                             uint8_t* queries_padded, const BfFastWs& ws, const BfOut& out, const BfScanEvents& ev,
                             hipStream_t s) {
    int* top8 = static_cast<int*>(ws.top8);
    int* thr = static_cast<int*>(ws.thr);
    int* tile_fail = ws.tile_fail(f);
    const BfGate failed{tile_fail, f.qg};
    hipError_t e;
    {
        const BfPlan& fb = f.fallback;
        uint32_t* gthr = reinterpret_cast<uint32_t*>(ws.fb.cnt + (size_t)fb.qpad * fb.nsplit);
        const size_t gwords = (size_t)fb.qpad + (size_t)fb.qpad * fb.nsplit;
        const size_t work = (size_t)f.qpad * 32 > gwords ? (size_t)f.qpad * 32 : gwords;
        size_t grid = (work + 255) / 256;
        if (grid > 2048) grid = 2048;
        hipLaunchKernelGGL(bf_u8_prep_kernel, dim3((unsigned)grid), dim3(256), 0, s, queries_raw, nq, queries_padded, f.qpad,
                           tile_fail, f.nqt, gthr, gwords);
        e = hipGetLastError();
        if (e != hipSuccess) return e;
    }
    auto scan = [&](const BfScanArgs& sa, int grid) -> hipError_t {
        const void* fn = f.qg == 4 ? (const void*)bf_scan_u8_kernel<4, false> : (const void*)bf_scan_u8_kernel<2, false>;
        hipError_t le = hipFuncSetAttribute(fn, hipFuncAttributeMaxDynamicSharedMemorySize, (int)f.lds_scan);
        if (le != hipSuccess) return le;
        if (f.qg == 4) hipLaunchKernelGGL((bf_scan_u8_kernel<4, false>), dim3(grid), dim3(256), f.lds_scan, s, sa);
        else hipLaunchKernelGGL((bf_scan_u8_kernel<2, false>), dim3(grid), dim3(256), f.lds_scan, s, sa);
        return hipGetLastError();
    };
    BfScanArgs sa{};
    sa.base_i8 = rows.i8;
    sa.auxh = rows.auxh;
    sa.queries = queries_padded;
    sa.n = rows.n;
    const int s_nqt = f.qpad / (BF_TQ * f.qg);
// ... 179 lines not shown
        switch (kch) {
            case 2: return sample ? go(bf_scan_bf16_kernel<MODE, true, 1, 4, 2>) : go(bf_scan_bf16_kernel<MODE, false, 1, 4, 2>);
            case 3: return sample ? go(bf_scan_bf16_kernel<MODE, true, 1, 4, 3>) : go(bf_scan_bf16_kernel<MODE, false, 1, 4, 3>);
            case 4: return sample ? go(bf_scan_bf16_kernel<MODE, true, 1, 4, 4>) : go(bf_scan_bf16_kernel<MODE, false, 1, 4, 4>);
            case 6: return sample ? go(bf_scan_bf16_kernel<MODE, true, 1, 4, 6>) : go(bf_scan_bf16_kernel<MODE, false, 1, 4, 6>);
            case 8: return sample ? go(bf_scan_bf16_kernel<MODE, true, 1, 4, 8>) : go(bf_scan_bf16_kernel<MODE, false, 1, 4, 8>);
            default: return hipErrorInvalidValue;
        }
    }
    const char* w8e = getenv("NMSLIB_GPU_BF16_W8");
    const int w8 = w8e ? atoi(w8e) : 7;
    if (sample) return (w8 & 4) ? launch_scan_bf16_one<MODE, true, 1, 8>(a, grid, lds, s) : launch_scan_bf16_one<MODE, true, 2, 4>(a, grid, lds, s);
    if (terms == 1) {
        if (qg == 2) return (w8 & 1) ? launch_scan_bf16_one<MODE, false, 2, 8>(a, grid, lds, s) : launch_scan_bf16_one<MODE, false, 4, 4>(a, grid, lds, s);
        return (w8 & 2) ? launch_scan_bf16_one<MODE, false, 1, 8>(a, grid, lds, s) : launch_scan_bf16_one<MODE, false, 2, 4>(a, grid, lds, s);
    }
    if (qg == 2) return launch_scan_f32_one<MODE, false, 4>(a, grid, lds, s);
    return launch_scan_f32_one<MODE, false, 2>(a, grid, lds, s);
}

static void dump_rerank_list_clocks(const unsigned long long* d_prof, hipStream_t s) {
    unsigned long long h[16];
    (void)hipStreamSynchronize(s);
    (void)hipMemcpy(h, d_prof, sizeof(h), hipMemcpyDeviceToHost);
    const double wg = h[10] ? (double)h[10] : 1.0;
    fprintf(stderr, "[rerank f32 list] workgroups %llu rows/query %.1f fetched/query %.1f P %.1f | us since start: prefix %.2f "
            "gather %.2f distances %.2f sort %.2f proof %.2f out %.2f\n", h[10], h[8] / wg, h[11] / wg, h[9] / wg, h[0] / wg / 100,
            h[1] / wg / 100, h[2] / wg / 100, h[3] / wg / 100, h[4] / wg / 100, h[5] / wg / 100);
}

static void dump_f32_fast_checksums(const BfF32Fast& f, const BfFastWs& ws, hipStream_t s) {
    (void)hipStreamSynchronize(s);
    auto sum = [&](const void* d, size_t bytes) -> unsigned long long {
        std::vector<uint32_t> h(bytes / 4);
        (void)hipMemcpy(h.data(), d, bytes, hipMemcpyDeviceToHost);
        unsigned long long x = 1469598103934665603ull;
        for (uint32_t v : h) x = (x ^ v) * 1099511628211ull;
        return x;
    };
    std::vector<int> cnt((size_t)f.qpad * f.nsplit * 2);
    (void)hipMemcpy(cnt.data(), ws.list_cnt, cnt.size() * 4, hipMemcpyDeviceToHost);
    std::vector<uint32_t> lst((size_t)f.qpad * f.nsplit * 2 * f.caph);
    (void)hipMemcpy(lst.data(), ws.list, lst.size() * 4, hipMemcpyDeviceToHost);
    unsigned long long lx = 1469598103934665603ull;
    long long rows = 0;
    const size_t nl = (size_t)f.nsplit * 2;
    for (size_t i = 0; i < cnt.size(); ++i) {
        rows += cnt[i];
        int have = 0;
        for (int j = 0; j < f.caph && have < cnt[i]; ++j) {
            const uint32_t e = lst[((i / nl) * f.caph + j) * nl + i % nl];
            lx = (lx ^ e) * 1099511628211ull;
            have += __builtin_popcount(e & 0xffffu);
        }
    }
    fprintf(stderr, "[f32fast] top8 %016llx thr %016llx thr1 %016llx flags %016llx cnt %016llx list %016llx rows %lld\n",
            sum(ws.top8, bf_fast_ws_bytes(f).top8), sum(ws.thr, (size_t)f.qpad * 4), sum(ws.thr1(f), (size_t)f.qpad * 4),
            sum(ws.tile_fail(f), (size_t)f.nqt * 8), sum(ws.list_cnt, cnt.size() * 4), lx, rows);
}

hipError_t launch_bf_f32_fast(const BfF32Fast& f, int space, int nq, int k, const BfF32Rows& rows, const BfF32Tiles& tiles,
                              const BfF32Queries& q, const BfFastWs& ws, const BfOut& out, const BfScanEvents& ev,
                              hipStream_t s) {
    const int sdim = f.cosc ? f.sel_dim : rows.dim, sld = f.cosc ? q.sel_ld : rows.ldb;
    float* top8 = static_cast<float*>(ws.top8);
    float* thr = static_cast<float*>(ws.thr);
    float* thr1 = ws.thr1(f);
    int* tile_fail = ws.tile_fail(f);
    int* precise = ws.precise(f);
    void* q_hi = ws.q_tile(f, BfFastWs::Q_HI);
    void* q_lo = ws.q_tile(f, BfFastWs::Q_LO);
    void* q_h16 = ws.q_tile(f, BfFastWs::Q_H16);
    hipError_t e;
    {
        const BfPlan& fb = f.fallback;
        uint32_t* gthr = reinterpret_cast<uint32_t*>(ws.fb.cnt + (size_t)fb.qpad * fb.nsplit);
        const size_t gwords = 2 * ((size_t)fb.qpad + (size_t)fb.qpad * fb.nsplit);
        size_t work = (size_t)f.qpad * f.dp > gwords ? (size_t)f.qpad * f.dp : gwords;
        size_t grid = (work + 255) / 256;
        if (grid > 2048) grid = 2048;
        hipLaunchKernelGGL(bf_f32_prep_kernel, dim3((unsigned)grid), dim3(256), 0, s, q.raw, nq, sdim, q.sel, f.qpad,
                           sld, q.raw ? q.padded : nullptr, f.kch > 1 ? nullptr : static_cast<__bf16*>(q_hi),
                           f.kch > 1 ? nullptr : static_cast<__bf16*>(q_lo),
                           tile_fail, 2 * f.nqt, ws.flags_fb, fb.nqt, gthr, gwords, f.dp, static_cast<_Float16*>(q_h16), q.scale_q);
        e = hipGetLastError();
        if (e != hipSuccess) return e;
    }
    auto scan = [&](const BfScanF32Args& sa, bool sample, int terms, int grid) -> hipError_t {
        const size_t lds = terms == 1 ? f.lds_scan1 : f.lds_scan;
        if (f.mode == 0) return launch_scan_f32_mode<SC_L2>(sa, sample, terms, f.qg, grid, lds, s, f.kch);
        if (f.mode == 1) return launch_scan_f32_mode<SC_DOT>(sa, sample, terms, f.qg, grid, lds, s, f.kch);
        return launch_scan_f32_mode<SC_COS>(sa, sample, terms, f.qg, grid, lds, s, f.kch);
    };
    BfScanF32Args a{};
    a.base_hi = static_cast<const __bf16*>(tiles.hi);
    a.base_lo = static_cast<const __bf16*>(tiles.lo);
    a.auxp = tiles.auxp;
    a.q_hi = static_cast<const __bf16*>(q_hi);
    a.q_lo = static_cast<const __bf16*>(q_lo);
    a.base_h16 = tiles.h16;
    {
        static const int prio = getenv("NMSLIB_GPU_BF16_PRIO") ? atoi(getenv("NMSLIB_GPU_BF16_PRIO")) : 0;
        a.prio_half = prio;
    }
    a.q_h16 = q_h16;
    a.auxp16 = tiles.auxp16;
    a.n = rows.n;
    a.nqt = f.nqt;
    BfScanF32Args sa = a;
    sa.nqt = f.qpad / (f.kch > 1 ? 128 : 256);
    sa.nsplit = f.s_nsplit;
    sa.tps = f.s_tps;
    sa.tile_stride = f.stride;
    sa.top8 = top8;
    e = scan(sa, true, 1, 8 * sa.nqt * (f.s_nsplit / 8));
    if (e != hipSuccess) return e;
    {
        static const bool dbg_nohit = getenv("NMSLIB_GPU_DEBUG") && (atoi(getenv("NMSLIB_GPU_DEBUG")) & 8192);
        const int depth = f.rcap <= 64 && f.s_nsplit >= 32 ? 4 : 8;
        const dim3 tgrid((f.qpad + 3) / 4);
#define BF_THR_ARGS                                                                                                               \
    top8, 2 * f.s_nsplit, depth, f.r, f.rcap, nq, f.qpad, q.sel, sld, sdim, tiles.scale * (f.mode == 2 ? 1.0f : tiles.bmax), tiles.bres16, f.tq, \
        f.force_precise ? 1 : (dbg_nohit ? 2 : 0), thr, thr1, precise, q.scale_q, tiles.scale * q.scale_q
        if (2 * f.s_nsplit * depth <= 512) hipLaunchKernelGGL(bf_f32_threshold_kernel<8>, tgrid, dim3(256), 0, s, BF_THR_ARGS);
        else hipLaunchKernelGGL(bf_f32_threshold_kernel<16>, tgrid, dim3(256), 0, s, BF_THR_ARGS);
#undef BF_THR_ARGS
    }
    e = hipGetLastError();
    if (e != hipSuccess) return e;
    a.list = ws.list;
    a.list_cnt = ws.list_cnt;
    a.nsplit = f.nsplit;
    a.tps = f.tps;
    a.caph = f.caph;
    a.tile_stride = 1;
    a.group_flag = precise;
    a.list_m_off = ws.list_m_off(f);
    const int grid = 8 * f.nqt * (f.nsplit / 8);
    if (ev.first) (void)hipEventRecord(ev.first, s);
    if (!f.force_precise) {
        a.thr = thr1;
        a.group_want = 0;
        e = scan(a, false, 1, grid);
        if (e != hipSuccess) return e;
    }
    a.thr = thr;
    a.group_want = 1;
    e = scan(a, false, 3, grid);
    if (ev.second) (void)hipEventRecord(ev.second, s);
    if (e != hipSuccess) return e;
    RerankListF32Args r{};
    r.base = rows.orig;
    r.queries = q.padded;
    r.list = ws.list;
    r.list_cnt = ws.list_cnt;
    r.ext_ids = out.ext_ids;
    r.out_ids = out.ids;
    r.out_dists = out.dists;
    r.out_cnt = out.cnt;
    r.tile_fail = tile_fail;
    r.n = rows.n;
    r.k = k;
    r.nsplit = f.nsplit;
    r.caph = f.caph;
    r.tps = f.tps;
    r.p2max = f.p2max;
    r.fail_queries = f.tq;
    r.no_split = f.kch > 1 ? 1 : 0;
    r.space = space;
    r.dim = rows.dim;
    r.ldb = rows.ldb;
    r.queries_sel = q.sel;
    r.sel_dim = sdim;
    r.sel_ld = sld;
    r.scale = tiles.scale;
    r.scale_q = q.scale_q;
    r.bres16 = tiles.bres16;
    r.qaux = f.cosc ? q.qaux_cosc : nullptr;
    r.thr = thr;
    r.thr1 = thr1;
    r.precise = precise;
    r.list_m_off = ws.list_m_off(f);
    r.bmax = tiles.bmax;
    r.bres = tiles.bres;
    static const int dbg = getenv("NMSLIB_GPU_DEBUG") ? atoi(getenv("NMSLIB_GPU_DEBUG")) : 0;
    static unsigned long long* d_prof = nullptr;
    if (dbg & 4096) {
        if (!d_prof) (void)hipMalloc(&d_prof, 16 * 8);
        (void)hipMemsetAsync(d_prof, 0, 16 * 8, s);
        r.prof = d_prof;
    }
    e = hipFuncSetAttribute(reinterpret_cast<const void*>(bf_rerank_f32_list_kernel),
                            hipFuncAttributeMaxDynamicSharedMemorySize, (int)f.lds_rerank);
    if (e != hipSuccess) return e;
    hipLaunchKernelGGL(bf_rerank_f32_list_kernel, dim3(nq), dim3(256), f.lds_rerank, s, r);
    e = hipGetLastError();
    if (e != hipSuccess) return e;
    if (dbg & 4096) dump_rerank_list_clocks(d_prof, s);
    if (dbg & 2048) dump_f32_fast_checksums(f, ws, s);
    BfF32Queries fq = q;
    fq.sel = f.cosc ? q.centred : q.sel;
    fq.qaux_cosc = f.cosc ? q.qaux_cosc : nullptr;
    return launch_bf_adaptive_f32(f.fallback, space, k, rows, fq, ws.fb, ws.flags_fb, BfGate{tile_fail, f.tq / 128}, out, s,
                                  true);
}

hipError_t launch_row_aux_f32(const float* base, int n, int ldb, int dim, int space, float* aux,
                              hipStream_t s) {
    if (n == 0) return hipSuccess;
    hipLaunchKernelGGL(row_aux_f32_kernel, dim3((n + 3) / 4), dim3(256), 0, s, base, n, ldb, dim, space, aux);
    return hipGetLastError();
}
hipError_t launch_prepare_u8(const uint8_t* base, int n, uint8_t* rows_i8, int32_t* aux, int32_t* auxh, hipStream_t s) {
    const int n_pad = bf_u8_rows_padded(n);
    hipLaunchKernelGGL(prepare_u8_kernel, dim3((n_pad + 3) / 4), dim3(256), 0, s, base, n, n_pad, rows_i8, aux, auxh);
    return hipGetLastError();
}
hipError_t launch_pad_rows(const void* src, int rows, int dim, void* dst, int rows_pad, int ld,
                           int elem_bytes, hipStream_t s) {
    const size_t total = (size_t)rows_pad * ld * elem_bytes;
    if (total == 0) return hipSuccess;
    int grid = (int)((total + 255) / 256);
    if (grid > 4096) grid = 4096;
    hipLaunchKernelGGL(pad_rows_kernel, dim3(grid), dim3(256), 0, s, (const uint8_t*)src, rows,
                       dim * elem_bytes, (uint8_t*)dst, rows_pad, ld * elem_bytes);
    return hipGetLastError();
}
hipError_t launch_normalize_rows(float* rows, int n, int ld, int dim, hipStream_t s) {
    if (n == 0) return hipSuccess;
    hipLaunchKernelGGL(normalize_rows_kernel, dim3((n + 3) / 4), dim3(256), 0, s, rows, n, ld, dim);
    return hipGetLastError();
}
hipError_t launch_row_aux_cosc(const float* orig, const float* centred, int n, int ldb, int dim, double mu_norm, float* aux,
                               hipStream_t s) {
    if (n == 0) return hipSuccess;
    hipLaunchKernelGGL(row_aux_cosc_kernel, dim3((n + 3) / 4), dim3(256), 0, s, orig, centred, n, ldb, dim, mu_norm, aux);
    return hipGetLastError();
}
hipError_t launch_query_aux_cosc(const float* orig, const float* centred, int nq, int ldb, int dim, double mu_norm,
                                 float* qaux, hipStream_t s) {
    if (nq == 0) return hipSuccess;
    hipLaunchKernelGGL(query_aux_cosc_kernel, dim3((nq + 3) / 4), dim3(256), 0, s, orig, centred, nq, ldb, dim, mu_norm,
                       qaux);
    return hipGetLastError();
}
hipError_t launch_row_aug_cosc(const float* orig, const float* centred, int n, int ldb, int dim, double mu_norm, float lambda,
                               float* out, int ldo, int* zero_rows, hipStream_t s) {
    if (n == 0) return hipSuccess;
    hipLaunchKernelGGL(row_aug_cosc_kernel, dim3((n + 3) / 4), dim3(256), 0, s, orig, centred, n, ldb, dim, mu_norm, lambda, out,
                       ldo, zero_rows);
    return hipGetLastError();
}
hipError_t launch_query_aug_cosc(const float* centred, const float* qaux, int nq, int qpad, int ldb, int dim, float lambda,
                                 float* out, int ldo, hipStream_t s) {
    if (qpad == 0) return hipSuccess;
    hipLaunchKernelGGL(query_aug_cosc_kernel, dim3((qpad + 3) / 4), dim3(256), 0, s, centred, qaux, nq, qpad, ldb, dim, lambda,
                       out, ldo);
    return hipGetLastError();
}
hipError_t launch_col_stats(const float* base, int n, int ldb, int dim, double* stats, hipStream_t s) {
    hipError_t e = hipMemsetAsync(stats, 0, ((size_t)ldb + 1) * 8, s);
    if (e != hipSuccess || n == 0) return e;
    int grid = (n + 255) / 256;
    if (grid > 2048) grid = 2048;
    const int rpb = (n + grid - 1) / grid;
    hipLaunchKernelGGL(col_stats_kernel, dim3(grid), dim3(256), 0, s, base, n, ldb, dim, rpb, stats);
    return hipGetLastError();
}
hipError_t launch_center_rows(const float* src, const float* mean, int rows, int rows_valid, int ld, int dim, float* dst,
                              hipStream_t s) {
    const size_t total = (size_t)rows * ld;
    if (total == 0) return hipSuccess;
    size_t grid = (total + 255) / 256;
    if (grid > 8192) grid = 8192;
    hipLaunchKernelGGL(center_rows_kernel, dim3((unsigned)grid), dim3(256), 0, s, src, mean, rows, rows_valid, ld, dim, dst);
    return hipGetLastError();
}
hipError_t launch_pair_distance(int space, const void* a, const void* b, int dim, float* out,
                                hipStream_t s) {
    hipLaunchKernelGGL(pair_distance_kernel, dim3(1), dim3(64), 0, s, space, a, b, dim, out);
    return hipGetLastError();
// ... 25 lines not shown
```

nmslib_zig_amd/csrc/kernels/kernels.hpp:

```cpp
#pragma once
#include <hip/hip_runtime_api.h>
#include <stddef.h>
#include <stdint.h>

#include <utility>

namespace gfxknn {

enum SpaceCode : int {
    SP_L2 = 0,
    SP_L1 = 1,
    SP_LINF = 2,
    SP_COSINE = 3,
    SP_ANGULAR = 4,
    SP_NEGDOT = 5,
    SP_L2SQR_SIFT = 6,
    SP_L2SQR = 7,
    SP_NORMCOS = 8,
    SP_QNORM_NEGDOT = 9,
    SP_LEVEN = 10,
    SP_BIT_HAMMING = 11,
    SP_KLDIV = 12,
    SP_KLDIV_RQ = 13,
    SP_KLDIVGEN = 14,
    SP_KLDIVGEN_RQ = 15,
    SP_KLDIVGEN_SLOW = 16,
    SP_ITAKURASAITO = 17,
    SP_JSDIV = 18,
    SP_JSDIV_SLOW = 19,
    SP_JSMETR = 20,
    SP_JSMETR_SLOW = 21,
};

constexpr int BF_TQ = 128;
constexpr int BF_BN = 64;
constexpr int BF_KC = 128;
constexpr int BF_MAX_K = 512;

struct BfPlan {
    int nq, qpad, nqt;
    int n;
    int ldb;
    int nsplit, rows_per_split;
    int kprime, cap;
    int p2max;
    int xj, xm;
    size_t lds_select, lds_rerank;
};
BfPlan bf_make_plan(int n, int dim, int nq, int k, bool is_u8, int qpad_multiple = BF_TQ);
inline size_t bf_cand_elems(const BfPlan& p) { return (size_t)p.qpad * p.nsplit * p.cap; }
inline size_t bf_cnt_elems(const BfPlan& p) { return 3 * (size_t)p.qpad * p.nsplit + 2 * (size_t)p.qpad; }

inline int f32_row_stride(int dim) { return (dim + 7) & ~7; }

hipError_t launch_row_aux_f32(const float* base, int n, int ldb, int dim, int space, float* aux,
                              hipStream_t s);
inline int bf_u8_rows_padded(int n) { return (n + BF_BN - 1) / BF_BN * BF_BN + BF_BN; }
hipError_t launch_prepare_u8(const uint8_t* base, int n, uint8_t* rows_i8, int32_t* aux, int32_t* auxh, hipStream_t s);
hipError_t launch_pad_rows(const void* src, int rows, int dim, void* dst, int rows_pad, int ld,
                           int elem_bytes, hipStream_t s);
hipError_t launch_normalize_rows(float* rows, int n, int ld, int dim, hipStream_t s);

hipError_t launch_col_stats(const float* base, int n, int ldb, int dim, double* stats, hipStream_t s);
hipError_t launch_center_rows(const float* src, const float* mean, int rows, int rows_valid, int ld, int dim, float* dst,
                              hipStream_t s);

hipError_t launch_row_aux_cosc(const float* orig, const float* centred, int n, int ldb, int dim, double mu_norm, float* aux,
                               hipStream_t s);
hipError_t launch_query_aux_cosc(const float* orig, const float* centred, int nq, int ldb, int dim, double mu_norm,
                                 float* qaux, hipStream_t s);

struct BfOut {
    const int32_t* ext_ids;
    int32_t* ids;
    float* dists;
    int32_t* cnt;
};
struct BfGate {
    const int* flags = nullptr;
    int tiles = 1;
};
struct BfCand {
    unsigned long long* cand;
    int* cnt;
};
struct BfVerify {
    int* flags = nullptr;
    const float* queries_sel = nullptr;
    float bmax = 0.f;
};
struct BfF32Rows {
    const float *orig, *sel, *aux;
    int n, dim, ldb;
    float bmax;
};
struct BfF32Queries {
    const float* raw;
    float* padded;
    const float* sel;
    const float* centred;
    const float* qaux_cosc;
    int sel_ld;
    float scale_q;
};
struct BfU8Rows {
    const uint8_t *orig, *i8;
    const int32_t *aux, *auxh;
    int n;
};
using BfScanEvents = std::pair<hipEvent_t, hipEvent_t>;

hipError_t launch_bf_select_u8(const BfPlan& p, const uint8_t* base_i8, const int32_t* aux, const uint8_t* queries_padded,
                               const BfCand& c, const BfGate& gate, hipStream_t s, bool cleared = false);
hipError_t launch_bf_select_direct_f32(const BfPlan& p, int space, const float* base, const float* queries_padded,
                                       const BfCand& c, const BfGate& gate, hipStream_t s,
                                       bool cleared_second_region = false);
hipError_t launch_bf_rerank(const BfPlan& p, int space, int dim, int k, const void* base, const void* queries_padded,
                            const BfCand& c, const BfGate& gate, const BfVerify& verify, const BfOut& out, hipStream_t s);
hipError_t launch_bf_adaptive_f32(const BfPlan& p, int space, int k, const BfF32Rows& rows, const BfF32Queries& q,
                                  const BfCand& c, int* flags, const BfGate& gate, const BfOut& out, hipStream_t s,
                                  bool cleared = false);

struct BfU8Fast {
    bool use;
    int qg;
    int qpad, nqt;
    int stride, r;
    int nsplit, tps, caph;
    int p2max;
    size_t lds_scan, lds_thr, lds_rerank;
    int s_nsplit, s_tps;
    BfPlan fallback;
};
BfU8Fast bf_u8_fast_plan(int n, int nq, int k);

struct BfF32Fast {
    bool use;
    int mode;
    int qg;
    bool cosc;
    int sel_dim;
    int kch;
    int dp;
    int tq;
    int qpad, nqt;
    int stride, r;
    int rcap;
    bool force_precise;
    int nsplit, tps, caph, p2max;
    int s_nsplit, s_tps;
    size_t lds_scan, lds_scan1, lds_thr, lds_rerank;
    BfPlan fallback;
};
BfF32Fast bf_f32_fast_plan(int n, int dim, int nq, int k, int space, bool cosine_centred);

struct BfFastWsBytes {
    size_t top8, thr, list, list_cnt, cand, cnt, flags_fb, queries;
};
inline BfFastWsBytes bf_fast_ws_bytes(const BfU8Fast& f) {
    const size_t lists = (size_t)f.qpad * f.nsplit * 2;
    return {(size_t)f.qpad * f.s_nsplit * 2 * 8 * 4, (size_t)f.qpad * 4 + (size_t)f.nqt * 4 + 64, lists * f.caph * 4, lists * 4,
            bf_cand_elems(f.fallback) * 8, bf_cnt_elems(f.fallback) * 4, 0, 0};
}
inline BfFastWsBytes bf_fast_ws_bytes(const BfF32Fast& f) {
    const size_t lists = (size_t)f.qpad * f.nsplit * 2;
    return {(size_t)f.qpad * f.s_nsplit * 2 * 8 * 4, (size_t)f.qpad * 8 + (size_t)f.nqt * 8 + 64, 2 * lists * f.caph * 4, lists * 4,
            bf_cand_elems(f.fallback) * 8, bf_cnt_elems(f.fallback) * 4, (size_t)f.fallback.nqt * 4 + 64,
            (size_t)f.qpad * f.dp * 2 * 3};
}
struct BfFastWs {
    void* top8;
    void* thr;
    uint32_t* list;
    int* list_cnt;
    BfCand fb;
    int* flags_fb;
    void* queries;

    size_t list_m_off(const BfF32Fast& f) const { return (size_t)f.qpad * f.caph * f.nsplit * 2; }
    int* tile_fail(const BfU8Fast& f) const { return static_cast<int*>(thr) + f.qpad; }
    float* thr1(const BfF32Fast& f) const { return static_cast<float*>(thr) + f.qpad; }
    int* tile_fail(const BfF32Fast& f) const { return reinterpret_cast<int*>(thr1(f) + f.qpad); }
    int* precise(const BfF32Fast& f) const { return tile_fail(f) + f.nqt; }
    enum QueryTile { Q_HI = 0, Q_LO = 1, Q_H16 = 2 };
    void* q_tile(const BfF32Fast& f, QueryTile t) const { return static_cast<char*>(queries) + (size_t)t * f.qpad * f.dp * 2; }
};

hipError_t launch_bf_u8_fast(const BfU8Fast& f, int nq, int k, const BfU8Rows& rows, const uint8_t* queries_raw,
                             uint8_t* queries_padded, const BfFastWs& ws, const BfOut& out, const BfScanEvents& ev,
                             hipStream_t s);

inline int bf_f32_rows_padded(int n) { return (n + BF_BN - 1) / BF_BN * BF_BN + BF_BN; }
hipError_t launch_row_maxnorm(const float* rows, int n, int ld, int dim, bool relative_residual, float* out, hipStream_t s,
                              float scale16 = 0.f);
struct BfF32Tiles {
    void *hi, *lo;
    float* auxp;
    void* h16;
    float* auxp16;
    float scale, bres16;
    int dp;
    float bmax, bres;
};
struct BfSplitSrc {
    const float* rows;
    int n, n_pad, ld, cols;
};
hipError_t launch_split_bf16(const BfSplitSrc& src, const float* aux, float aux_pad, float aux16_mul, const BfF32Tiles& dst,
                             hipStream_t s);
hipError_t launch_bf_f32_fast(const BfF32Fast& f, int space, int nq, int k, const BfF32Rows& rows, const BfF32Tiles& tiles,
                              const BfF32Queries& q, const BfFastWs& ws, const BfOut& out, const BfScanEvents& ev,
                              hipStream_t s);
hipError_t launch_row_aug_cosc(const float* orig, const float* centred, int n, int ldb, int dim, double mu_norm, float lambda,
                               float* out, int ldo, int* zero_rows, hipStream_t s);
hipError_t launch_query_aug_cosc(const float* centred, const float* qaux, int nq, int qpad, int ldb, int dim, float lambda,
                                 float* out, int ldo, hipStream_t s);

constexpr int BF_L1_MAX_DIM = 256;
constexpr int BF_L1_ROW_TILE = 128;
inline int bf_l1_rows_padded(int n) { return (n + BF_L1_ROW_TILE - 1) / BF_L1_ROW_TILE * BF_L1_ROW_TILE; }
struct BfL1Fast {
    bool use;
    int d4;
    int qpad, nqt;
    int nsplit, rows_per_split;
    int kprime;
    size_t lds_scan;
    BfPlan list;
    BfPlan fallback;
};
BfL1Fast bf_l1_fast_plan(int n, int dim, int nq, int k);
struct BfL1Rows {
    const uint32_t* u8;
    const float *lo, *hi, *rmax;
    double step;
};
struct BfL1Ws {
    uint32_t* qt;
    double* xe;
    BfCand cand;
    int* flags;
    BfCand fb;
};
hipError_t launch_l1_col_range(const float* rows, int n, int ld, int dim, uint32_t* range, hipStream_t s);
hipError_t launch_l1_quantise_rows(const float* rows, int n, int ld, int dim, const float* lo, double step, uint32_t* out,
                                   uint32_t* rmax_bits, hipStream_t s);
hipError_t launch_bf_l1_fast(const BfL1Fast& f, int nq, int k, const BfF32Rows& rows, const BfL1Rows& copy,
                             const float* queries_raw, float* queries_padded, const BfL1Ws& ws, const BfOut& out,
                             const BfScanEvents& ev, hipStream_t s);

// ... 243 lines not shown
```

Baseline: 3.061 million.

## Fuse brute-force select, rerank and exact fallback into one persistent tail kernel

Adds a persistent work-queue kernel that runs the select, rerank, exact re-select and final rerank phases of the adaptive f32 brute-force path. Blocks take tickets from a global counter and wait on per-tile completion counters, so dependent phases can overlap across tiles instead of being separated by kernel launches. It is on by default (NMSLIB_GPU_TAIL=1) and includes a spin-wait timeout whose count is exposed through a new stats field. In exchange it adds inter-block spin dependencies, a grid capped by occupancy, and a risk of stalls or timeouts.

```diff
diff --git a/include/nmslib_gpu.h b/include/nmslib_gpu.h
--- a/include/nmslib_gpu.h
+++ b/include/nmslib_gpu.h
@@ -45,6 +45,7 @@
     size_t fast_tiles_precise;
     size_t fast_tiles_fallback;
     size_t hnsw_redone;
+    size_t bf_tail_timeouts;
 } nmslib_gpu_stats_t;
 nmslib_error_t nmslib_gpu_get_stats(nmslib_index_handle_t index, nmslib_gpu_stats_t* out);
 
diff --git a/nmslib_zig_amd/__init__.py b/nmslib_zig_amd/__init__.py
--- a/nmslib_zig_amd/__init__.py
+++ b/nmslib_zig_amd/__init__.py
@@ -75,7 +75,8 @@
     _fields_ = [("upload_seconds", C.c_double), ("build_seconds", C.c_double),
                 ("hbm_bytes", C.c_size_t), ("rows", C.c_size_t), ("dim", C.c_size_t), ("shards", C.c_size_t),
                 ("last_path", C.c_size_t), ("fast_tiles", C.c_size_t), ("fast_tiles_precise", C.c_size_t),
-                ("fast_tiles_fallback", C.c_size_t), ("hnsw_redone", C.c_size_t)]
+                ("fast_tiles_fallback", C.c_size_t), ("hnsw_redone", C.c_size_t),
+                ("bf_tail_timeouts", C.c_size_t)]
 
 
 def build_library(force=False):
diff --git a/nmslib_zig_amd/csrc/abi.cpp b/nmslib_zig_amd/csrc/abi.cpp
--- a/nmslib_zig_amd/csrc/abi.cpp
+++ b/nmslib_zig_amd/csrc/abi.cpp
@@ -824,6 +824,7 @@
         out->last_path = (size_t)e->last_path;
         e->fast_tile_counts(&out->fast_tiles, &out->fast_tiles_precise, &out->fast_tiles_fallback);
         out->hnsw_redone = e->hnsw_redone();
+        out->bf_tail_timeouts = e->bf_tail_timeouts();
     });
 }
 
diff --git a/nmslib_zig_amd/csrc/brute.cpp b/nmslib_zig_amd/csrc/brute.cpp
--- a/nmslib_zig_amd/csrc/brute.cpp
+++ b/nmslib_zig_amd/csrc/brute.cpp
@@ -232,6 +232,7 @@
                        hipStream_t stream) {
     BruteDense& b = brute_;
     have_counters_ = false;
+    tail_timeouts_ = nullptr;
     const int dim_eff = d_n_ ? (int)dim_ : 1;
     const BfOut out{d_ids_.as<int32_t>(), d_ids, d_dists, d_cnt};
     if (k > (size_t)BF_MAX_K) {
@@ -319,6 +320,7 @@
             fast_flags_ = ws.tile_fail(f);
             fast_nqt_ = f.nqt;
             fast_has_precise_ = true;
+            tail_timeouts_ = bf_tail_timeout_word(f.fallback, ws.flags_fb);
             return;
         }
     }
@@ -376,7 +378,8 @@
     } else if (space_ == SP_L1 || space_ == SP_LINF) {
         hip_check(launch_bf_select_direct_f32(p, space_, rows.orig, q.padded, c, BfGate{}, stream), "bf_select_direct");
     } else {
-        b.ws_flags.ensure((size_t)p.nqt * 4 + 64);
+        b.ws_flags.ensure(bf_adaptive_flag_words(p) * 4);
+        if (space_ == SP_L2 && rows.bmax > 0.f) tail_timeouts_ = bf_tail_timeout_word(p, b.ws_flags.as<int>());
         hip_check(launch_bf_adaptive_f32(p, space_, (int)k, rows, q, c, b.ws_flags.as<int>(), BfGate{}, out, stream),
                   "bf_adaptive_f32");
         prof_end(stream);
diff --git a/nmslib_zig_amd/csrc/engine.cpp b/nmslib_zig_amd/csrc/engine.cpp
--- a/nmslib_zig_amd/csrc/engine.cpp
+++ b/nmslib_zig_amd/csrc/engine.cpp
@@ -316,6 +316,7 @@
     last_path = 0;
     fast_flags_ = nullptr;
     fast_nqt_ = 0;
+    tail_timeouts_ = nullptr;
     hnsw_fix_valid_ = false;
     have_counters_ = false;
     d_rows16_.release();
@@ -1115,6 +1116,16 @@
     }
 }
 
+size_t Engine::bf_tail_timeouts() {
+    if (!shards_.empty()) return shards_[0]->bf_tail_timeouts();
+    if ((last_path != 0 && last_path != 1) || !tail_timeouts_) return 0;
+    int v = 0;
+    hip_check(hipSetDevice(device_), "hipSetDevice");
+    hip_check(hipStreamSynchronize(last_stream_ ? last_stream_ : stream_), "stats");
+    hip_check(hipMemcpy(&v, tail_timeouts_, 4, hipMemcpyDeviceToHost), "stats tail timeouts");
+    return (size_t)v;
+}
+
 size_t Engine::hnsw_redone() {
     if (!shards_.empty()) return shards_[0]->hnsw_redone();
     if ((last_path != 4 && last_path != 5) || !hnsw_fix_valid_) return 0;
diff --git a/nmslib_zig_amd/csrc/engine.hpp b/nmslib_zig_amd/csrc/engine.hpp
--- a/nmslib_zig_amd/csrc/engine.hpp
+++ b/nmslib_zig_amd/csrc/engine.hpp
@@ -217,6 +217,8 @@
     const int* fast_flags_ = nullptr;
     int fast_nqt_ = 0;
     bool fast_has_precise_ = false;
+    const int* tail_timeouts_ = nullptr;
+    size_t bf_tail_timeouts();
     void fast_tile_counts(size_t* tiles, size_t* precise, size_t* fallback);
     size_t hnsw_redone();
     hipStream_t last_stream_ = nullptr;
diff --git a/nmslib_zig_amd/csrc/kernels/bf_kernels.hip b/nmslib_zig_amd/csrc/kernels/bf_kernels.hip
--- a/nmslib_zig_amd/csrc/kernels/bf_kernels.hip
+++ b/nmslib_zig_amd/csrc/kernels/bf_kernels.hip
@@ -1,3 +1,4 @@
+#include <cstddef>
 #include <cstdio>
 #include <type_traits>
 #include <vector>
@@ -190,13 +191,11 @@
 __device__ long long g_bf_trace[2048][3];
 
 template <int MODE, bool FULL, bool ONE>
-__global__ __launch_bounds__(256, 2) void bf_select_f32_kernel(BfArgs a) {
-    extern __shared__ __attribute__((aligned(16))) char smem[];
+__device__ __forceinline__ void bf_select_f32_body(const BfArgs a, const int b, char* smem) {
     const int tid = threadIdx.x, lane = tid & 63, wave = tid >> 6;
     const long long clk_c0 = __builtin_readcyclecounter(), clk_r0 = wall_clock64();
     const int h = lane >> 5, l31 = lane & 31;
 
-    const int b = blockIdx.x;
     const int xcd = b & 7, rest = b >> 3;
     const int qt = rest % a.nqt;
     const int split = (rest / a.nqt) * 8 + xcd;
@@ -592,16 +591,22 @@
     }
     if (h == 0) a.cand_cnt[(size_t)qidx * a.nsplit + split] = mycnt;
     if ((a.dbg & 1024) && tid == 0) {
-        if (blockIdx.x == 0) {
+        if (b == 0) {
             g_bf_clk[0] = __builtin_readcyclecounter() - clk_c0;
             g_bf_clk[1] = wall_clock64() - clk_r0;
         }
-        if (blockIdx.x < 2048) {
-            g_bf_trace[blockIdx.x][0] = clk_r0;
-            g_bf_trace[blockIdx.x][1] = wall_clock64();
-            g_bf_trace[blockIdx.x][2] = __builtin_amdgcn_s_getreg((4 << 0) | (0 << 6) | (31 << 11));
-        }
-    }
+        if (b < 2048) {
+            g_bf_trace[b][0] = clk_r0;
+            g_bf_trace[b][1] = wall_clock64();
+            g_bf_trace[b][2] = __builtin_amdgcn_s_getreg((4 << 0) | (0 << 6) | (31 << 11));
+        }
+    }
+}
+
+template <int MODE, bool FULL, bool ONE>
+__global__ __launch_bounds__(256, 2) void bf_select_f32_kernel(BfArgs a) {
+    extern __shared__ __attribute__((aligned(16))) char smem[];
+    bf_select_f32_body<MODE, FULL, ONE>(a, blockIdx.x, smem);
 }
 
 struct BfArgsU8 {
@@ -2425,11 +2430,10 @@
     float eps_rel;
 };
 
-__global__ __launch_bounds__(256) void bf_rerank_kernel(RerankArgs a) {
-    extern __shared__ __attribute__((aligned(16))) char smem[];
+__device__ __forceinline__ void bf_rerank_body(const RerankArgs a, const int q, char* smem, uint32_t* kth_word, float* qn2_word) {
     u64* keys = reinterpret_cast<u64*>(smem);
     int* offs = reinterpret_cast<int*>(keys + a.p2max);
-    const int q = blockIdx.x, tid = threadIdx.x, lane = tid & 63, wave = tid >> 6;
+    const int tid = threadIdx.x, lane = tid & 63, wave = tid >> 6;
     if (a.tile_fail && a.tile_fail[q / a.fail_queries] == 0) return;
 
     if (tid == 0) {
@@ -2443,7 +2447,7 @@
     }
     __syncthreads();
     const int total = offs[a.nsplit];
-    __shared__ uint32_t s_kth;
+    uint32_t& s_kth = *kth_word;
     const bool verify = a.verify_flags != nullptr && a.space == SP_L2 && total >= a.kprime;
     if (tid == 0) s_kth = 0xffffffffu;
     for (int idx = tid; idx < a.nsplit * a.kprime; idx += blockDim.x) {
@@ -2520,7 +2524,7 @@
     }
     if (tid == 0 && a.out_cnt) a.out_cnt[q] = found;
     if (verify && found > 0) {
-        __shared__ float s_qn2v;
+        float& s_qn2v = *qn2_word;
         if (tid < 64) {
             const float* qs = a.queries_sel + (size_t)q * a.ldb;
             float ss = 0.f;
@@ -2536,6 +2540,161 @@
             const float e = a.eps_rel * (qn * a.bmax + 0.5f * a.bmax * a.bmax);
             const float floor_d2 = qn2 - 2.0f * kth - 2.0f * e - 2e-6f * (qn2 + fabsf(kth));
             if (!(dk * dk <= floor_d2)) atomicOr(&a.verify_flags[q / a.verify_queries], 1);
+        }
+    }
+}
+
+__global__ __launch_bounds__(256) void bf_rerank_kernel(RerankArgs a) {
+    extern __shared__ __attribute__((aligned(16))) char smem[];
+    __shared__ uint32_t s_kth;
+    __shared__ float s_qn2v;
+    bf_rerank_body(a, blockIdx.x, smem, &s_kth, &s_qn2v);
+}
+
+struct BfTailArgs {
+    BfArgs sel;
+    BfArgs exact;
+    RerankArgs rr;
+    const int* gate;
+    uint32_t* state;
+    BfTailShape shape;
+    int lds_main;
+    int force_verify;
+    long long spin_ticks;
+};
+
+__device__ __forceinline__ bool bf_tail_wait(uint32_t* counter, uint32_t full, uint32_t* tmo, long long ticks) {
+    const long long t0 = wall_clock64();
+    for (;;) {
+        if (__hip_atomic_load(counter, __ATOMIC_RELAXED, __HIP_MEMORY_SCOPE_AGENT) >= full) return true;
+        if (__hip_atomic_load(tmo, __ATOMIC_RELAXED, __HIP_MEMORY_SCOPE_AGENT) != 0u) return false;
+        if (wall_clock64() - t0 > ticks) {
+            __hip_atomic_fetch_add(tmo, 1u, __ATOMIC_RELAXED, __HIP_MEMORY_SCOPE_AGENT);
+            return false;
+        }
+        __builtin_amdgcn_s_sleep(16);
+    }
+}
+
+template <typename T>
+__device__ __forceinline__ T tail_arg(size_t offset) {
+    static_assert(sizeof(T) % 4 == 0, "whole words");
+    const __attribute__((address_space(4))) uint32_t* kp =
+        (const __attribute__((address_space(4))) uint32_t*)__builtin_amdgcn_kernarg_segment_ptr();
+    asm volatile("" : "+s"(kp));
+    union {
+        T v;
+        uint32_t w[sizeof(T) / 4];
+    } u;
+#pragma unroll
+    for (size_t i = 0; i < sizeof(T) / 4; ++i) u.w[i] = kp[offset / 4 + i];
+    return u.v;
+}
+
+__device__ __forceinline__ int* tail_ctl(char* smem) { return reinterpret_cast<int*>(smem + tail_arg<int>(offsetof(BfTailArgs, lds_main))); }
+
+struct BfTailNow {
+    BfTailShape sh;
+    unsigned total;
+    bool any;
+    BfTailTask task;
+};
+__device__ __forceinline__ BfTailNow tail_now(char* smem) {
+    auto uni = [](int v) __attribute__((always_inline)) { return __builtin_amdgcn_readfirstlane(v); };
+    const int* ctl = tail_ctl(smem);
+    BfTailNow n;
+    n.sh = tail_arg<BfTailShape>(offsetof(BfTailArgs, shape));
+    BfTailCounts c;
+    c.nopen = uni(ctl[4]), c.nfull = uni(ctl[5]), c.part = uni(ctl[6]);
+    c.per_select = (unsigned)uni(ctl[7]), c.per_rerank = (unsigned)uni(ctl[8]), c.total = (unsigned)uni(ctl[9]);
+    const unsigned ticket = (unsigned)uni(ctl[0]);
+    n.total = c.total;
+    n.any = ticket < c.total;
+    n.task = BfTailTask{};
+    if (n.any) {
+        n.task = bf_tail_task(n.sh, c, ctl + 12, ticket);
+        n.task.tile = uni(n.task.tile);
+    }
+    return n;
+}
+
+template <int MODE, bool FULL, bool ONE>
+__global__ __launch_bounds__(256, 2) void bf_tail_kernel(BfTailArgs a) {
+    const int tid = threadIdx.x, lane = tid & 63;
+    if (a.gate) {
+        const int nflags = (a.shape.nqt + a.shape.group - 1) / a.shape.group;
+        bool open = false;
+        for (int i = lane; i < nflags; i += 64) open |= a.gate[i] != 0;
+        if (!__any(open)) return;
+    }
+    extern __shared__ __attribute__((aligned(16))) char smem[];
+    {
+        int* ctl = reinterpret_cast<int*>(smem + a.lds_main);
+        if (tid == 0) *reinterpret_cast<BfTailCounts*>(ctl + 4) = bf_tail_open(a.shape, a.gate, ctl + 12);
+    }
+    for (;;) {
+        __syncthreads();
+        if (tid == 0) {
+            int* ctl = tail_ctl(smem);
+            uint32_t* state = tail_arg<uint32_t*>(offsetof(BfTailArgs, state));
+            unsigned t = (unsigned)ctl[9];
+            if (__hip_atomic_load(state + BF_TAIL_TIMEOUT, __ATOMIC_RELAXED, __HIP_MEMORY_SCOPE_AGENT) == 0u)
+                t = __hip_atomic_fetch_add(state + BF_TAIL_TICKET, 1u, __ATOMIC_RELAXED, __HIP_MEMORY_SCOPE_AGENT);
+            ctl[0] = (int)t;
+        }
+        __syncthreads();
+        {
+            const BfTailNow n = tail_now(smem);
+            if (!n.any) break;
+            const BfTailTask task = n.task;
+            if (task.phase > n.sh.first) {
+                int* ctl = tail_ctl(smem);
+                if (tid == 0) {
+                    uint32_t* state = tail_arg<uint32_t*>(offsetof(BfTailArgs, state));
+                    const bool ok = bf_tail_wait(state + bf_tail_counter(n.sh, task.phase - 1, task.tile),
+                                                 bf_tail_full(n.sh, task.phase - 1, task.tile), state + BF_TAIL_TIMEOUT,
+                                                 tail_arg<long long>(offsetof(BfTailArgs, spin_ticks)));
+                    if (ok) __builtin_amdgcn_fence(__ATOMIC_ACQUIRE, "agent");
+                    asm volatile("s_waitcnt vmcnt(0)" ::: "memory");
+                    ctl[1] = ok ? 1 : 0;
+                }
+                __syncthreads();
+                if (__builtin_amdgcn_readfirstlane(ctl[1]) == 0) break;
+            }
+            int* verify_flags = tail_arg<int*>(offsetof(BfTailArgs, rr) + offsetof(RerankArgs, verify_flags));
+            bool run = true;
+            if (task.phase >= 2)
+                run = __builtin_amdgcn_readfirstlane(
+                          __hip_atomic_load(verify_flags + task.tile, __ATOMIC_RELAXED, __HIP_MEMORY_SCOPE_AGENT)) != 0;
+            if (run) {
+                if (bf_tail_selects(task.phase)) {
+                    const int b = ((task.item >> 3) * n.sh.nqt + task.tile) * 8 + (task.item & 7);
+                    if (task.phase == 0) bf_select_f32_body<MODE, FULL, ONE>(tail_arg<BfArgs>(offsetof(BfTailArgs, sel)), b, smem);
+                    else if constexpr (MODE == BF_L2)
+                        bf_select_f32_body<BF_L2D, false, false>(tail_arg<BfArgs>(offsetof(BfTailArgs, exact)), b, smem);
+                } else {
+                    RerankArgs r = tail_arg<RerankArgs>(offsetof(BfTailArgs, rr));
+                    if (task.phase != 1) r.verify_flags = nullptr;
+                    int* ctl = tail_ctl(smem);
+                    bf_rerank_body(r, task.tile * n.sh.tq + task.item, smem, reinterpret_cast<uint32_t*>(ctl + 2),
+                                   reinterpret_cast<float*>(ctl + 3));
+                }
+            }
+        }
+        const BfTailNow n = tail_now(smem);
+        if (n.task.phase == 1 && tid == 0 && tail_arg<int>(offsetof(BfTailArgs, force_verify))) {
+            int* verify_flags = tail_arg<int*>(offsetof(BfTailArgs, rr) + offsetof(RerankArgs, verify_flags));
+            if (verify_flags) atomicOr(&verify_flags[n.task.tile], 1);
+        }
+        if (n.task.phase < n.sh.last) {
+            asm volatile("s_waitcnt vmcnt(0)" ::: "memory");
+            __syncthreads();
+            if (tid == 0) {
+                __builtin_amdgcn_fence(__ATOMIC_RELEASE, "agent");
+                asm volatile("s_waitcnt vmcnt(0)" ::: "memory");
+                __hip_atomic_fetch_add(tail_arg<uint32_t*>(offsetof(BfTailArgs, state)) + bf_tail_counter(n.sh, n.task.phase, n.task.tile),
+                                       1u, __ATOMIC_RELAXED, __HIP_MEMORY_SCOPE_AGENT);
+            }
         }
     }
 }
@@ -2847,6 +3006,11 @@
         __syncthreads();
         if (threadIdx.x == 0) cnt_out[q] = total < k ? total : k;
     }
+}
+
+static int env_now(const char* name, int otherwise) {
+    const char* e = getenv(name);
+    return e ? atoi(e) : otherwise;
 }
 
 static int host_next_pow2(int v) {
@@ -2899,7 +3063,39 @@
 }
 
 template <int MODE, bool FULL, bool ONE>
-static hipError_t launch_select_kern(const BfPlan& p, const BfArgs& a, hipStream_t s) {
+static hipError_t launch_tail_kern(const BfPlan& p, const BfArgs& sel, const BfTailArgs& tail, hipStream_t s) {
+    auto kern = bf_tail_kernel<MODE, FULL, ONE>;
+    BfTailArgs a = tail;
+    a.sel = sel;
+    a.sel.tile_fail = nullptr;
+    const size_t lds_main = ((p.lds_select > p.lds_rerank ? p.lds_select : p.lds_rerank) + 15) / 16 * 16;
+    const size_t lds = lds_main + 48 + (size_t)p.nqt * 4;
+    a.lds_main = (int)lds_main;
+    hipError_t e = hipFuncSetAttribute(reinterpret_cast<const void*>(kern), hipFuncAttributeMaxDynamicSharedMemorySize, (int)lds);
+    if (e != hipSuccess) return e;
+    static size_t occ_lds = 0;
+    static int occ_grid = 0;
+    if (occ_lds != lds) {
+        int dev = 0, cus = 0, per_cu = 0;
+        if ((e = hipGetDevice(&dev)) != hipSuccess) return e;
+        if ((e = hipDeviceGetAttribute(&cus, hipDeviceAttributeMultiprocessorCount, dev)) != hipSuccess) return e;
+        if ((e = hipOccupancyMaxActiveBlocksPerMultiprocessor(&per_cu, kern, 256, lds)) != hipSuccess) return e;
+        if (per_cu < 1 || cus < 1) return hipErrorInvalidConfiguration;
+        occ_grid = cus * (per_cu < 2 ? per_cu : 2);
+        occ_lds = lds;
+    }
+    static const int want = getenv("NMSLIB_GPU_TAIL_GRID") ? atoi(getenv("NMSLIB_GPU_TAIL_GRID")) : 512;
+    int grid = want < occ_grid ? want : occ_grid;
+    if (grid < 1) grid = 1;
+    hipLaunchKernelGGL(kern, dim3(grid), dim3(256), lds, s, a);
+    return hipGetLastError();
+}
+
+template <int MODE, bool FULL, bool ONE>
+static hipError_t launch_select_kern(const BfPlan& p, const BfArgs& a, hipStream_t s, const BfTailArgs* tail) {
+    if constexpr (MODE == BF_L2 || MODE == BF_DOT || MODE == BF_COS || MODE == BF_COSC) {
+        if (tail) return launch_tail_kern<MODE, FULL, ONE>(p, a, *tail, s);
+    }
     auto kern = bf_select_f32_kernel<MODE, FULL, ONE>;
     hipError_t e = hipFuncSetAttribute(reinterpret_cast<const void*>(kern),
                                        hipFuncAttributeMaxDynamicSharedMemorySize, (int)p.lds_select);
@@ -2931,17 +3127,17 @@
 }
 
 template <int MODE>
-static hipError_t launch_select_mode(const BfPlan& p, const BfArgs& a, hipStream_t s) {
+static hipError_t launch_select_mode(const BfPlan& p, const BfArgs& a, hipStream_t s, const BfTailArgs* tail = nullptr) {
 #ifdef BF_FAST_COMPILE
-    if (MODE == BF_L2 && p.ldb == BF_KC) return launch_select_kern<BF_L2, true, true>(p, a, s);
+    if (MODE == BF_L2 && p.ldb == BF_KC) return launch_select_kern<BF_L2, true, true>(p, a, s, tail);
     return hipErrorInvalidValue;
 #else
     if constexpr (MODE == BF_L1 || MODE == BF_LINF || MODE == BF_L2D) {
-        return launch_select_kern<MODE, false, false>(p, a, s);
+        return launch_select_kern<MODE, false, false>(p, a, s, tail);
     } else {
-        if (p.ldb == BF_KC) return launch_select_kern<MODE, true, true>(p, a, s);
-        if (p.ldb % BF_KC == 0) return launch_select_kern<MODE, true, false>(p, a, s);
-        return launch_select_kern<MODE, false, false>(p, a, s);
+        if (p.ldb == BF_KC) return launch_select_kern<MODE, true, true>(p, a, s, tail);
+        if (p.ldb % BF_KC == 0) return launch_select_kern<MODE, true, false>(p, a, s, tail);
+        return launch_select_kern<MODE, false, false>(p, a, s, tail);
     }
 #endif
 }
@@ -2970,29 +3166,30 @@
     a.kcs = p.ldb < BF_KC ? p.ldb : BF_KC;
     a.nchunks = (p.ldb + BF_KC - 1) / BF_KC;
     static const int dbg = getenv("NMSLIB_GPU_DEBUG") ? atoi(getenv("NMSLIB_GPU_DEBUG")) : 0;
-    a.dbg = dbg;
+    a.dbg = dbg & ~(16384 | 32768);
     return a;
 }
 
 static hipError_t select_f32(const BfPlan& p, int space, const float* base, const float* aux, const float* queries_padded,
-                             const float* qaux_cosc, const BfCand& c, const BfGate& gate, hipStream_t s, bool cleared) {
+                             const float* qaux_cosc, const BfCand& c, const BfGate& gate, hipStream_t s, bool cleared,
+                             int regions = 1, const BfTailArgs* tail = nullptr) {
     uint32_t* gthr = reinterpret_cast<uint32_t*>(c.cnt + (size_t)p.qpad * p.nsplit);
     if (!cleared) {
-        hipError_t me = hipMemsetAsync(gthr, 0, ((size_t)p.qpad + (size_t)p.qpad * p.nsplit) * 4, s);
+        hipError_t me = hipMemsetAsync(gthr, 0, regions * ((size_t)p.qpad + (size_t)p.qpad * p.nsplit) * 4, s);
         if (me != hipSuccess) return me;
     }
     BfArgs a = make_args(p, base, aux, queries_padded, c, gate, gthr);
     switch (space) {
-        case SP_L2: return launch_select_mode<BF_L2>(p, a, s);
-        case SP_NEGDOT: return launch_select_mode<BF_DOT>(p, a, s);
+        case SP_L2: return launch_select_mode<BF_L2>(p, a, s, tail);
+        case SP_NEGDOT: return launch_select_mode<BF_DOT>(p, a, s, tail);
         case SP_COSINE:
         case SP_ANGULAR:
             if (qaux_cosc) {
                 a.qaux = qaux_cosc;
                 a.aux_stride = p.n;
-                return launch_select_mode<BF_COSC>(p, a, s);
-            }
-            return launch_select_mode<BF_COS>(p, a, s);
+                return launch_select_mode<BF_COSC>(p, a, s, tail);
+            }
+            return launch_select_mode<BF_COS>(p, a, s, tail);
         default: return hipErrorInvalidValue;
     }
 }
@@ -3049,8 +3246,8 @@
     return hipGetLastError();
 }
 
-hipError_t launch_bf_rerank(const BfPlan& p, int space, int dim, int k, const void* base, const void* queries_padded,
-                            const BfCand& c, const BfGate& gate, const BfVerify& verify, const BfOut& out, hipStream_t s) {
+static RerankArgs make_rerank_args(const BfPlan& p, int space, int dim, int k, const void* base, const void* queries_padded,
+                                   const BfCand& c, const BfGate& gate, const BfVerify& verify, const BfOut& out) {
     RerankArgs a{};
     a.verify_flags = verify.flags;
     a.verify_queries = BF_TQ;
@@ -3075,6 +3272,12 @@
     a.cap = p.cap;
     a.kprime = p.kprime;
     a.p2max = p.p2max;
+    return a;
+}
+
+hipError_t launch_bf_rerank(const BfPlan& p, int space, int dim, int k, const void* base, const void* queries_padded,
+                            const BfCand& c, const BfGate& gate, const BfVerify& verify, const BfOut& out, hipStream_t s) {
+    const RerankArgs a = make_rerank_args(p, space, dim, k, base, queries_padded, c, gate, verify, out);
     hipError_t e = hipFuncSetAttribute(reinterpret_cast<const void*>(bf_rerank_kernel),
                                        hipFuncAttributeMaxDynamicSharedMemorySize, (int)p.lds_rerank);
     if (e != hipSuccess) return e;
@@ -3085,16 +3288,41 @@
 hipError_t launch_bf_adaptive_f32(const BfPlan& p, int space, int k, const BfF32Rows& rows, const BfF32Queries& q,
                                   const BfCand& c, int* flags, const BfGate& gate, const BfOut& out, hipStream_t s,
                                   bool cleared) {
-    hipError_t e = select_f32(p, space, rows.sel, rows.aux, q.sel, q.qaux_cosc, c, gate, s, cleared);
+    const bool one_tail = env_now("NMSLIB_GPU_TAIL", 1) != 0;
+    const int dbg = env_now("NMSLIB_GPU_DEBUG", 0);
+    const bool verify = space == SP_L2 && flags != nullptr && rows.bmax > 0.f;
+    const bool tail = one_tail && flags != nullptr && (verify || gate.flags);
+    const BfVerify proof = verify ? BfVerify{flags, q.sel, rows.bmax} : BfVerify{};
+    BfTailArgs t{};
+    if (tail) {
+        const size_t gwords = (size_t)p.qpad + (size_t)p.qpad * p.nsplit;
+        uint32_t* gthr2 = reinterpret_cast<uint32_t*>(c.cnt + (size_t)p.qpad * p.nsplit) + gwords;
+        t.exact = make_args(p, rows.orig, nullptr, q.padded, c, BfGate{}, gthr2);
+        t.rr = make_rerank_args(p, space, rows.dim, k, rows.orig, q.padded, c, BfGate{}, proof, out);
+        t.gate = gate.flags;
+        t.state = reinterpret_cast<uint32_t*>(flags) + bf_tail_state_offset(p);
+        t.shape = BfTailShape{p.nqt, BF_TQ, p.nq, p.nsplit, gate.tiles, gate.flags ? 0 : 2, verify ? 3 : 1};
+        t.force_verify = (dbg & 32768) != 0;
+        t.spin_ticks = 400000000ll;
+    }
+    hipError_t e;
+    if (tail && gate.flags) {
+        if (!cleared) {
+            e = hipMemsetAsync(flags, 0, bf_adaptive_flag_words(p) * 4, s);
+            if (e != hipSuccess) return e;
+        }
+        return select_f32(p, space, rows.sel, rows.aux, q.sel, q.qaux_cosc, c, BfGate{}, s, cleared, 2, &t);
+    }
+    e = select_f32(p, space, rows.sel, rows.aux, q.sel, q.qaux_cosc, c, gate, s, cleared, tail ? 2 : 1);
     if (e != hipSuccess) return e;
-    const bool verify = space == SP_L2 && flags != nullptr && rows.bmax > 0.f;
     if (!verify) return launch_bf_rerank(p, space, rows.dim, k, rows.orig, q.padded, c, gate, BfVerify{}, out, s);
     if (!cleared) {
-        e = hipMemsetAsync(flags, 0, (size_t)p.nqt * 4, s);
+        e = hipMemsetAsync(flags, 0, bf_adaptive_flag_words(p) * 4, s);
         if (e != hipSuccess) return e;
     }
-    e = launch_bf_rerank(p, space, rows.dim, k, rows.orig, q.padded, c, gate, BfVerify{flags, q.sel, rows.bmax}, out, s);
+    e = launch_bf_rerank(p, space, rows.dim, k, rows.orig, q.padded, c, gate, proof, out, s);
     if (e != hipSuccess) return e;
+    if (tail) return select_f32(p, space, rows.sel, rows.aux, q.sel, q.qaux_cosc, c, BfGate{}, s, true, 1, &t);
     const BfGate failed{flags, 1};
     e = launch_bf_select_direct_f32(p, SP_L2, rows.orig, q.padded, c, failed, s, cleared);
     if (e != hipSuccess) return e;
@@ -3440,7 +3668,8 @@
         hipLaunchKernelGGL(bf_f32_prep_kernel, dim3((unsigned)grid), dim3(256), 0, s, q.raw, nq, sdim, q.sel, f.qpad,
                            sld, q.raw ? q.padded : nullptr, f.kch > 1 ? nullptr : static_cast<__bf16*>(q_hi),
                            f.kch > 1 ? nullptr : static_cast<__bf16*>(q_lo),
-                           tile_fail, 2 * f.nqt, ws.flags_fb, fb.nqt, gthr, gwords, f.dp, static_cast<_Float16*>(q_h16), q.scale_q);
+                           tile_fail, 2 * f.nqt, ws.flags_fb, (int)bf_adaptive_flag_words(fb), gthr, gwords, f.dp,
+                           static_cast<_Float16*>(q_h16), q.scale_q);
         e = hipGetLastError();
         if (e != hipSuccess) return e;
     }
@@ -3555,6 +3784,10 @@
     e = hipGetLastError();
     if (e != hipSuccess) return e;
     if (dbg & 4096) dump_rerank_list_clocks(d_prof, s);
+    if (env_now("NMSLIB_GPU_DEBUG", 0) & 16384) {
+        e = hipMemsetD32Async(reinterpret_cast<hipDeviceptr_t>(tile_fail), 1, (size_t)f.nqt, s);
+        if (e != hipSuccess) return e;
+    }
     if (dbg & 2048) dump_f32_fast_checksums(f, ws, s);
     BfF32Queries fq = q;
     fq.sel = f.cosc ? q.centred : q.sel;
diff --git a/nmslib_zig_amd/csrc/kernels/bf_tail_plan.hpp b/nmslib_zig_amd/csrc/kernels/bf_tail_plan.hpp
--- /dev/null
+++ b/nmslib_zig_amd/csrc/kernels/bf_tail_plan.hpp
@@ -0,0 +1,85 @@
+#pragma once
+
+#if defined(__HIPCC__) || defined(__CUDACC__)
+#define BF_TAIL_FN __host__ __device__ inline
+#else
+#define BF_TAIL_FN inline
+#endif
+
+namespace gfxknn {
+
+struct BfTailShape {
+    int nqt;
+    int tq;
+    int nq;
+    int nsplit;
+    int group;
+    int first, last;
+};
+
+struct BfTailCounts {
+    int nopen;
+    int nfull;
+    int part;
+    unsigned per_select, per_rerank, total;
+};
+
+struct BfTailTask {
+    int phase, tile, item;
+};
+
+enum : int { BF_TAIL_TICKET = 0, BF_TAIL_TIMEOUT = 1, BF_TAIL_HEAD = 4 };
+BF_TAIL_FN int bf_tail_state_words(int nqt, int phases) { return BF_TAIL_HEAD + (phases - 1) * nqt; }
+BF_TAIL_FN int bf_tail_counter(const BfTailShape& s, int phase, int tile) { return BF_TAIL_HEAD + (phase - s.first) * s.nqt + tile; }
+
+BF_TAIL_FN bool bf_tail_selects(int phase) { return (phase & 1) == 0; }
+
+BF_TAIL_FN int bf_tail_tile_queries(const BfTailShape& s, int tile) {
+    const long long left = (long long)s.nq - (long long)tile * s.tq;
+    return left <= 0 ? 0 : (left < s.tq ? (int)left : s.tq);
+}
+
+BF_TAIL_FN BfTailCounts bf_tail_open(const BfTailShape& s, const int* flags, int* list) {
+    BfTailCounts c{};
+    for (int t = 0; t < s.nqt; ++t) {
+        const int nqs = bf_tail_tile_queries(s, t);
+        if (nqs == 0) break;
+        if (flags && flags[t / s.group] == 0) continue;
+        list[c.nopen++] = t;
+        if (nqs == s.tq) c.nfull++;
+        else c.part = nqs;
+    }
+    c.per_select = (unsigned)c.nopen * (unsigned)s.nsplit;
+    c.per_rerank = (unsigned)c.nfull * (unsigned)s.tq + (unsigned)c.part;
+    c.total = 0;
+    for (int p = s.first; p <= s.last; ++p) c.total += bf_tail_selects(p) ? c.per_select : c.per_rerank;
+    return c;
+}
+
+BF_TAIL_FN unsigned bf_tail_full(const BfTailShape& s, int phase, int tile) {
+    return bf_tail_selects(phase) ? (unsigned)s.nsplit : (unsigned)bf_tail_tile_queries(s, tile);
+}
+
+BF_TAIL_FN BfTailTask bf_tail_task(const BfTailShape& s, const BfTailCounts& c, const int* list, unsigned ticket) {
+    BfTailTask t{};
+    int phase = s.first;
+    for (;; ++phase) {
+        const unsigned n = bf_tail_selects(phase) ? c.per_select : c.per_rerank;
+        if (ticket < n) break;
+        ticket -= n;
+    }
+    t.phase = phase;
+    if (bf_tail_selects(phase)) {
+        const unsigned rest = ticket >> 3;
+        t.tile = list[rest % (unsigned)c.nopen];
+        t.item = (int)(rest / (unsigned)c.nopen) * 8 + (int)(ticket & 7u);
+    } else {
+        const unsigned full = (unsigned)c.nfull * (unsigned)s.tq;
+        const int slot = ticket < full ? (int)(ticket / (unsigned)s.tq) : c.nfull;
+        t.tile = list[slot];
+        t.item = (int)(ticket - (unsigned)slot * (unsigned)s.tq);
+    }
+    return t;
+}
+
+}
diff --git a/nmslib_zig_amd/csrc/kernels/kernels.hpp b/nmslib_zig_amd/csrc/kernels/kernels.hpp
--- a/nmslib_zig_amd/csrc/kernels/kernels.hpp
+++ b/nmslib_zig_amd/csrc/kernels/kernels.hpp
@@ -4,6 +4,8 @@
 #include <stdint.h>
 
 #include <utility>
+
+#include "bf_tail_plan.hpp"
 
 namespace gfxknn {
 
@@ -51,6 +53,12 @@
 inline size_t bf_cand_elems(const BfPlan& p) { return (size_t)p.qpad * p.nsplit * p.cap; }
 inline size_t bf_cnt_elems(const BfPlan& p) { return 3 * (size_t)p.qpad * p.nsplit + 2 * (size_t)p.qpad; }
 
+inline size_t bf_tail_state_offset(const BfPlan& p) { return ((size_t)p.nqt + 3) / 4 * 4; }
+inline const int* bf_tail_timeout_word(const BfPlan& p, const int* flags) { return flags + bf_tail_state_offset(p) + BF_TAIL_TIMEOUT; }
+inline size_t bf_adaptive_flag_words(const BfPlan& p) {
+    return bf_tail_state_offset(p) + ((size_t)bf_tail_state_words(p.nqt, 4) + 3) / 4 * 4;
+}
+
 inline int f32_row_stride(int dim) { return (dim + 7) & ~7; }
 
 hipError_t launch_row_aux_f32(const float* base, int n, int ldb, int dim, int space, float* aux,
@@ -165,7 +173,7 @@
 inline BfFastWsBytes bf_fast_ws_bytes(const BfF32Fast& f) {
     const size_t lists = (size_t)f.qpad * f.nsplit * 2;
     return {(size_t)f.qpad * f.s_nsplit * 2 * 8 * 4, (size_t)f.qpad * 8 + (size_t)f.nqt * 8 + 64, 2 * lists * f.caph * 4, lists * 4,
-            bf_cand_elems(f.fallback) * 8, bf_cnt_elems(f.fallback) * 4, (size_t)f.fallback.nqt * 4 + 64,
+            bf_cand_elems(f.fallback) * 8, bf_cnt_elems(f.fallback) * 4, bf_adaptive_flag_words(f.fallback) * 4,
             (size_t)f.qpad * f.dp * 2 * 3};
 }
 struct BfFastWs {
```

Result: no change. 3.055 million (-0.2%).
